# jovoy/SolarAxionRayTracing

Hardware: AMD Instinct MI355X
Metric: rays/sec (higher is better)
Workload: dtype f64

## Files before the change

### solaraxionraytracing_amd/csrc/sart_angular_scan.inc

```
  struct LdsLayout {
    TablesLds S;
    double cells[kRingExtraCells];
    DevBlob B;
    TraceArgs Ab;
    QueueLds<BLOCK / 64> Q;
  };
  __shared__ LdsLayout lds;
  static_assert((offsetof(LdsLayout, Q) % 512) == 0, "the rings are addressed with ds_*2st64 offsets");
  static_assert(kAScanCells == (BLOCK / 64) * kQueue, "the per-angle cells are the u5 column of the workgroup's rings");
  TablesLds& S = lds.S;
  QueueLds<BLOCK / 64>& Q = lds.Q;
  uint32_t* const cnt = reinterpret_cast<uint32_t*>(&lds.cells[kAScanCounters]);
  [[maybe_unused]] uint32_t* const cnt_out = reinterpret_cast<uint32_t*>(&lds.cells[kAImgNOutside]);
  auto acc_cell = [&](uint32_t t) -> double* { return &Q.w[t >> 7].u5[t & 127u]; };
  DevBlob& B = lds.B;
  TraceArgs& Ab = lds.Ab;
  (void)img_partials; (void)HBarg;
  {
    const uint64_t* src = reinterpret_cast<const uint64_t*>(blob);
    uint64_t* dst = reinterpret_cast<uint64_t*>(&B);
    for (int i = threadIdx.x; i < (int)(sizeof(DevBlob) / 8); i += BLOCK) dst[i] = src[i];
    if (threadIdx.x == 0) Ab = A;
    uint64_t* q = reinterpret_cast<uint64_t*>(&Q);
    for (int i = threadIdx.x; i < (int)(sizeof(Q) / 8); i += BLOCK) q[i] = 0ull;
// ... 128 lines not shown
    asm volatile("" :: "s"(HB.cdf_hi32), "s"(HB.energy_guide), "s"(HB.energy_tab), "s"(HB.refl), "s"(HB.refl_n_angles), "s"(HB.cdf_stride));
    RayOut out;
    phase_b<false, FAST, GAS, false, false, true>(Bo.P, L, HB, lds_opaque(Ab), st, e_idx, valid, out, nullptr);
    SART_STAGE_MARK("ACC");
    __builtin_amdgcn_s_setprio(SART_PRIO_ACC);
    if (__builtin_amdgcn_inverse_ballot_w64(out.m_nickel)) atomicAdd(&cnt[4 * kl + 1], 1u);
    if (__builtin_amdgcn_inverse_ballot_w64(out.m_till)) atomicAdd(&cnt[4 * kl + 2], 1u);
    if (out.passed) {
      atomicAdd(&cnt[4 * kl], 1u);
      double* const cell = acc_cell(kl * (2u * kScanLanes) + ((uint32_t)lane & (kScanLanes - 1u)));
      if constexpr (FIXED) {
        double fx_w, fx_w2;
        { const TraceArgs& Al = lds_opaque(Ab); fx_w = Al.fx_scale_w; fx_w2 = Al.fx_scale_w2; }
        __hip_atomic_fetch_add(reinterpret_cast<unsigned long long*>(cell), (unsigned long long)to_fixed(out.weight, fx_w), __ATOMIC_RELAXED,
                               __HIP_MEMORY_SCOPE_WORKGROUP);
        __hip_atomic_fetch_add(reinterpret_cast<unsigned long long*>(cell + kScanLanes), (unsigned long long)to_fixed(out.weight * out.weight, fx_w2),
                               __ATOMIC_RELAXED, __HIP_MEMORY_SCOPE_WORKGROUP);
      } else {
        __hip_atomic_fetch_add(cell, out.weight, __ATOMIC_RELAXED, __HIP_MEMORY_SCOPE_WORKGROUP);
        __hip_atomic_fetch_add(cell + kScanLanes, out.weight * out.weight, __ATOMIC_RELAXED, __HIP_MEMORY_SCOPE_WORKGROUP);
      }
      if constexpr (IMAGES) {
        SART_STAGE_MARK("IMG");
        TraceArgs Al;
        reload_kernarg(Al, offsetof(AScanKernArgs, A));
        asm volatile("" :: "s"(Al.replicas), "s"(Al.replica_stride), "s"(Al.image_nx), "s"(Al.image_ny), "s"(Al.image_x_min),
                     "s"(Al.image_y_min), "s"(Al.image_inv_step_x), "s"(Al.image_inv_step_y), "s"(Al.spectra));
        double* const blk = Al.replicas + (size_t)kl * (size_t)Al.replica_stride;
        double* const pos = &lds.cells[kAImgPos + kl * (3u * kAImgLanes) + ((uint32_t)lane & (kAImgLanes - 1u))];
        long long w_fx = 0;
        if constexpr (FIXED) {
          w_fx = to_fixed(out.weight, Al.fx_scale_w);
          __hip_atomic_fetch_add(reinterpret_cast<unsigned long long*>(pos), (unsigned long long)to_fixed(out.px, kFixedPositionScale),
                                 __ATOMIC_RELAXED, __HIP_MEMORY_SCOPE_WORKGROUP);
          __hip_atomic_fetch_add(reinterpret_cast<unsigned long long*>(pos + kAImgLanes), (unsigned long long)to_fixed(out.py, kFixedPositionScale),
                                 __ATOMIC_RELAXED, __HIP_MEMORY_SCOPE_WORKGROUP);
          __hip_atomic_fetch_add(reinterpret_cast<unsigned long long*>(pos + 2 * kAImgLanes), (unsigned long long)to_fixed(out.rdet, kFixedPositionScale),
                                 __ATOMIC_RELAXED, __HIP_MEMORY_SCOPE_WORKGROUP);
        } else {
          __hip_atomic_fetch_add(pos, out.px, __ATOMIC_RELAXED, __HIP_MEMORY_SCOPE_WORKGROUP);
          __hip_atomic_fetch_add(pos + kAImgLanes, out.py, __ATOMIC_RELAXED, __HIP_MEMORY_SCOPE_WORKGROUP);
          __hip_atomic_fetch_add(pos + 2 * kAImgLanes, out.rdet, __ATOMIC_RELAXED, __HIP_MEMORY_SCOPE_WORKGROUP);
        }
        const double fx = (out.px - Al.image_x_min) * Al.image_inv_step_x;
        const double fy = (out.py - Al.image_y_min) * Al.image_inv_step_y;
        const int nx = Al.image_nx, ny = Al.image_ny;
        const uint64_t inside_m = ballot64(fx >= 0.0) & ballot64(fx < (double)nx) & ballot64(fy >= 0.0) & ballot64(fy < (double)ny);
        if (__builtin_amdgcn_inverse_ballot_w64(inside_m)) {
          const uint32_t pix = (uint32_t)(int)fy * (uint32_t)nx + (uint32_t)(int)fx;
          if constexpr (FIXED) atomic_add_slot_i64(blk + pix, w_fx);
          else unsafeAtomicAdd(blk + pix, out.weight);
        } else {
          asm volatile("; rare: passed rays outside the image");
          atomicAdd(&cnt_out[kl], 1u);
          if constexpr (FIXED)
            __hip_atomic_fetch_add(reinterpret_cast<unsigned long long*>(&lds.cells[kAImgOutside + kl]), (unsigned long long)w_fx,
                                   __ATOMIC_RELAXED, __HIP_MEMORY_SCOPE_WORKGROUP);
        }
        if (Al.spectra) {
          double* rad = blk + (size_t)nx * (size_t)ny + SART_ACC_COUNT;
          double* en = rad + 2 * (size_t)Al.n_radial_bins;
          const size_t ne1 = (size_t)Pb.n_energies + 1;
          const int rb = min((int)(out.rdet * Al.radial_inv_bin), Al.n_radial_bins - 1);
          if constexpr (FIXED) {
            atomic_add_slot_i64(&rad[rb], 1);
            atomic_add_slot_i64(&rad[(size_t)Al.n_radial_bins + rb], w_fx);
            atomic_add_slot_i64(&en[out.e_idx], 1);
            atomic_add_slot_i64(&en[ne1 + out.e_idx], w_fx);
            atomic_add_slot_i64(&en[2 * ne1 + out.e_idx], to_fixed(out.reflect, kFixedReflectScale));
          } else {
            unsafeAtomicAdd(&rad[rb], 1.0);
            unsafeAtomicAdd(&rad[(size_t)Al.n_radial_bins + rb], out.weight);
            unsafeAtomicAdd(&en[out.e_idx], 1.0);
            unsafeAtomicAdd(&en[ne1 + out.e_idx], out.weight);
            unsafeAtomicAdd(&en[2 * ne1 + out.e_idx], out.reflect);
          }
        }
      }
    }
    __builtin_amdgcn_s_setprio(0);
  };

  constexpr bool kZonesInVgprs = FAST;
  uint32_t zone_lo_v[kMaxZones], zone_hi_v[kMaxZones];
#pragma unroll
  for (int z = 0; z < kMaxZones; ++z) {
    zone_lo_v[z] = H.zone_lo[z];
    zone_hi_v[z] = H.zone_hi[z];
    if (kZonesInVgprs) asm volatile("" : "+v"(zone_lo_v[z]), "+v"(zone_hi_v[z]));
  }
  uint32_t zone_reached_v = H.zone_reached;
  if (kZonesInVgprs) asm volatile("" : "+v"(zone_reached_v));
  uint32_t chunk = (uint32_t)wave_global;
  const uint32_t lane4 = 4u * (uint32_t)lane;
  uint32_t pass = 0;
  U4 stream = U4{0u, 0u, 0u, 0u};
  for (;;) {
    const bool have_new = chunk < n_chunks;
    SART_STAGE_MARK("LOOP");
    if (ka == n_angles) {
      if (have_new) {
        SART_STAGE_MARK("A0");
        if (pass == 0u) stream = stream_block(((first_chunk + (uint64_t)chunk) << 6) + (uint64_t)lane, A.seed_lo, A.seed_hi);
        const uint32_t w = word_of(stream, pass);
        const uint32_t rel = ((chunk << 8) + pass) + lane4;
        pass = (pass + 1u) & 3u;
        if (pass == 0u) chunk += (uint32_t)waves_total;
        if (early_reject) {
          ZoneTable Z;
          if constexpr (!kZonesInVgprs) reload_zones(Z);
          const uint32_t zone_reached = kZonesInVgprs ? (uint32_t)__builtin_amdgcn_readfirstlane((int)zone_reached_v) : Z.zone_reached;
          uint64_t dead_m = 0, reached_m = 0;
#pragma unroll
          for (int z = 0; z < kMaxZones; ++z) {
            const uint64_t in = kZonesInVgprs ? (ballot64(w >= zone_lo_v[z]) & ballot64(w <= zone_hi_v[z]))
                                              : (ballot64(w >= Z.lo[z]) & ballot64(w <= Z.hi[z]));
            dead_m |= in;
            reached_m |= ((zone_reached >> z) & 1u) ? in : 0ull;
          }
          const uint64_t valid_m = ballot64(rel >= rel_begin) & ballot64(rel < rel_end);
          n_reached += (uint32_t)__popcll(valid_m & reached_m);
          const uint64_t mask = valid_m & ~dead_m;
          if (__builtin_amdgcn_inverse_ballot_w64(mask)) {
            asm volatile("; hot: ring 0 write");
            const uint32_t slot = (t0 + prefix_of(mask)) % kQueue;
            Q.w[wave].ray[slot] = rel;
            Q.w[wave].u3hi[slot] = w;
          }
          t0 += (uint32_t)__popcll(mask);
          ring_sync();
        } else {
          run_bore(rel, (rel >= rel_begin) & (rel < rel_end), w);
        }
      }
      SART_STAGE_MARK("LOOP");
      if (early_reject) {
        const uint32_t n0 = t0 - h0;
        if ((n0 >= 64u) | (!have_new & (n0 > 0u))) {
          const uint32_t m = min(n0, 64u);
          const uint32_t slot = (h0 + (uint32_t)lane) % kQueue;
          const uint32_t rel = Q.w[wave].ray[slot];
          const uint32_t w = Q.w[wave].u3hi[slot];
          h0 += m;
          run_bore(rel, (uint32_t)lane < m, w);
        }
      }
    }
    SART_STAGE_MARK("LOOP");
    if (ka < n_angles) {
      run_telescope(ka);
      ++ka;
      ring_sync();
    }
    SART_STAGE_MARK("LOOP");
    const uint32_t n1 = t1 - h1;
    const bool draining = !have_new & (t0 == h0) & (ka == n_angles);
    if ((n1 >= 64u) | (draining & (n1 > 0u))) {
      run_mirrors(min(n1, 64u));
      ring_sync();
    }
    if (draining & (t1 == h1)) break;
  }

  SART_STAGE_MARK("EPILOGUE");
  if (lane == 0) atomicAdd(&cnt[4 * kAScanMaxAngles], n_reached);
  __syncthreads();
  using Sum = std::conditional_t<FIXED, long long, double>;
  for (int k = wave; k < n_angles; k += BLOCK / 64) {
    Sum* const dst = reinterpret_cast<Sum*>(ANarg.partials) + ((size_t)blockIdx.x * kAScanMaxAngles + (size_t)k) * kAScanPartialSlots;
    const double cell = *acc_cell((uint32_t)(k * 64 + lane));
    Sum v;
    if constexpr (FIXED) v = __double_as_longlong(cell); else v = cell;
#pragma unroll
    for (int off = 16; off > 0; off >>= 1) v += __shfl_xor(v, off, 64);
    if (lane == 0) dst[0] = v;
    if (lane == 32) dst[1] = v;
    if (lane < 4) dst[2 + lane] = (Sum)cnt[4 * k + lane];
    if (lane == 4) dst[6] = (k == 0) ? (Sum)cnt[4 * kAScanMaxAngles] : (Sum)0;
    if (lane == 5) dst[7] = (Sum)0;
    if constexpr (IMAGES) {
      const double pc = (lane < 3 * kAImgLanes) ? lds.cells[kAImgPos + k * (3 * kAImgLanes) + lane] : 0.0;
      Sum p;
      if constexpr (FIXED) p = __double_as_longlong(pc); else p = pc;
#pragma unroll
      for (int off = kAImgLanes / 2; off > 0; off >>= 1) p += __shfl_xor(p, off, 64);
      const Sum sw = __shfl(v, 0, 64), sw2 = __shfl(v, 32, 64);
      const Sum sx = __shfl(p, 0, 64), sy = __shfl(p, kAImgLanes, 64), sr = __shfl(p, 2 * kAImgLanes, 64);
      Sum s = 0;
      switch (lane) {
        case SART_ACC_SUM_WEIGHTS: s = sw; break;
        case SART_ACC_SUM_WEIGHTS_SQ: s = sw2; break;
        case SART_ACC_SUM_X: s = sx; break;
        case SART_ACC_SUM_Y: s = sy; break;
        case SART_ACC_SUM_R: s = sr; break;
        case SART_ACC_N_PASSED: s = (Sum)cnt[4 * k]; break;
        case SART_ACC_N_HIT_NICKEL: s = (Sum)cnt[4 * k + 1]; break;
        case SART_ACC_N_PASSED_TILL_WINDOW: s = (Sum)cnt[4 * k + 2]; break;
        case SART_ACC_N_SHELL_SELECTED: s = (Sum)cnt[4 * k + 3]; break;
        case SART_ACC_N_REACHED_TELESCOPE: s = (Sum)cnt[4 * kAScanMaxAngles]; break;
        case SART_ACC_N_OUTSIDE_IMAGE: s = (Sum)cnt_out[k]; break;
        case SART_ACC_SUM_WEIGHTS_OUTSIDE: if constexpr (FIXED) s = __double_as_longlong(lds.cells[kAImgOutside + k]); break;
        default: break;
// ... 5 lines not shown
```

### solaraxionraytracing_amd/csrc/sart_api.hip

```cpp
#include <hip/hip_runtime.h>
#include <rccl/rccl.h>
#include <dlfcn.h>
#include <sys/mman.h>
#include <unistd.h>

#include <algorithm>
#include <atomic>
#include <cmath>
#include <condition_variable>
#include <thread>
#include <cstdio>
#include <cstdlib>
#include <cstring>
#include <limits>
#include <map>
#include <mutex>
#include <string>
#include <vector>

#include "../../include/sart.h"
#include "sart_device.h"

namespace sart {
void launch_trace_histogram(const HotA& H, const HotB& HB, const DevBlob* blob, const TraceArgs& A, double* acc, int n_blocks,
                            hipStream_t stream, int variant, bool fixed);
void launch_finalize_fixed(const void* in, const void* hi, double* out, size_t n_img, int spectra, int n_radial_bins, int n_energies1, double q_w,
                           double q_w2, double q_pos, double q_refl, void* check_dev, hipStream_t stream);
void launch_rollover_fixed(void* acc, void* hi, size_t n, void* check_dev, hipStream_t stream);
size_t fixed_check_bytes();
std::string fixed_check_describe(const void* host_copy);
bool launch_trace_mass_scan(const HotA& H, const HotB& HB, const DevBlob* blob, const TraceArgs& A, const ScanArgs& SC, double* rows,
                            double* shared_row, int n_blocks, hipStream_t stream, int variant, bool fixed);
void launch_finalize_scan(const void* in, double* out, int n_masses, const double* q_w, const double* q_w2, int shared_row,
                          void* check_dev, hipStream_t stream, uint32_t counter_slots);
bool launch_trace_mass_scan_spectra(const HotA& H, const HotB& HB, const DevBlob* blob, const TraceArgs& A, const ScanArgs& SC, double* rows,
                                    double* shared_row, double* block0, double* counts, int n_blocks, hipStream_t stream, int variant, bool fixed);
int mass_scan_spectra_blocks_per_cu(int variant);
void launch_finalize_scan_bands(const void* rows, const void* shared_row, const void* in, double* out, const void* counts_in, double* counts_out,
                                int n_masses, int n_cells, const double* q_w, const double* q_w2, void* check_dev, hipStream_t stream);
void launch_trace_angular_scan(const HotA& H, const HotB& HB, const DevBlob* blob, const TraceArgs& A, const AScanArgs& AN, double* img_partials,
                               double* rows, double* shared_row, int n_blocks, hipStream_t stream, bool images, bool fast, bool fixed);
int angular_scan_blocks_per_cu(bool images, bool fast);
int energy_scan_blocks_per_cu(bool rotated);
void launch_trace_energy_scan(const HotA& H, const HotB& HB, const DevBlob* blob, const TraceArgs& A, const EScanArgs& EN, double* rows,
                              double* shared_row, int n_blocks, hipStream_t stream, bool rotated, bool fixed);
int shell_histogram_blocks_per_cu(bool rotated);
void launch_shell_histogram(const HotA& H, const HotB& HB, const DevBlob* blob, const TraceArgs& A, double* acc, const ShellArgs& SH,
                            int n_blocks, hipStream_t stream, bool rotated, bool fixed);
void launch_finalize_shells(const void* in, double* out, int n_shells, int n_energies1, int spectra, double q_w, double q_w2,
                            void* check_dev, hipStream_t stream);
int channel_histogram_blocks_per_cu(bool rotated);
void launch_channel_histogram(const HotA& H, const HotB& HB, const DevBlob* blob, const TraceArgs& A, double* acc, const ChannelArgs& CH,
                              int n_blocks, hipStream_t stream, bool rotated, bool fixed);
void launch_finalize_channels(const void* in, double* out, int n_channels, int n_energies1, int spectra, size_t n_img, double q_w,
                              double q_w2, void* check_dev, hipStream_t stream);
void launch_channel_fractions(const double* rates_dev, const double* total_dev, double* frac_dev, int n_channels, int stride,
                              size_t n_cells, unsigned long long* first_bad_dev, hipStream_t stream);
int origin_histogram_blocks_per_cu(bool rotated);
void launch_origin_histogram(const HotA& H, const HotB& HB, const DevBlob* blob, const TraceArgs& A, double* acc, const OriginArgs& OG,
                             int n_blocks, hipStream_t stream, bool rotated, bool fixed);
void launch_finalize_origin(const void* in, double* out, size_t n_cells, double q_w, double q_w2, void* check_dev, hipStream_t stream);
int aperture_histogram_blocks_per_cu(bool rotated);
void launch_aperture_histogram(const HotA& H, const HotB& HB, const DevBlob* blob, const TraceArgs& A, double* acc, const ApertureArgs& AP,
                               int n_blocks, hipStream_t stream, bool rotated, bool fixed);
int histogram_block_of(int variant);
void launch_trace_records(const HotA& H, const HotB& HB, const DevBlob* blob, const TraceArgs& A, sart_axion_t* out, int n_blocks,
                          hipStream_t stream, const double* uniforms_dev);
void launch_mirror_miss_count(const HotA& H, const DevBlob* blob, const TraceArgs& A, unsigned long long* counts, int n_blocks, hipStream_t stream);
void launch_radial_verdicts(const HotA& H, const DevBlob* blob, const double* radii, int n, uint32_t* out_table, uint32_t* out_compares,
                            hipStream_t stream);
int records_block();
int compact_chunk_max();
void launch_compact_records(const sart_axion_t* rec, uint32_t n, sart_axion_t* out, unsigned long long capacity, uint32_t* block_counts,
                            unsigned long long* block_first, unsigned long long* counts, hipStream_t stream);
void launch_stage_columns(const HotA& H, const HotB& HB, const DevBlob* blob, const TraceArgs& A, uint64_t* stage, uint32_t* flags,
                          uint32_t mask, int n_blocks, hipStream_t stream);
void launch_compact_columns(const uint64_t* stage, const uint32_t* flags, uint32_t n, uint32_t mask, unsigned long long ray_id0, uint64_t* out,
                            unsigned long long capacity, uint32_t* block_counts, unsigned long long* block_first,
                            unsigned long long* counts, hipStream_t stream);
int histogram_blocks_per_cu(int variant);
void launch_build_solar_tables(const double* em_dev, const double* radii_dev, const double* energies_dev, int n_radii, int n_energies,
                               double* cdf_dev, double* row_sum_dev, double* rcdf_dev, uint16_t* rguide_dev, uint16_t* eguide_dev,
                               uint32_t* status_dev, hipStream_t stream);
void launch_cdf_hi32(const double* cdf_dev, uint32_t* out_dev, size_t n, hipStream_t stream);
}

using namespace sart;

namespace {

thread_local std::string g_err;
int fail(int code, const std::string& msg) {
  g_err = msg;
  return code;
}
#define SART_HIP(call)                                                                              \
  do {                                                                                              \
    hipError_t e_ = (call);                                                                         \
    if (e_ != hipSuccess)                                                                           \
      return fail(e_ == hipErrorOutOfMemory ? SART_ERR_OUT_OF_MEMORY : SART_ERR_NO_DEVICE,          \
                  std::string(#call) + ": " + hipGetErrorString(e_));                               \
  } while (0)

constexpr double kPi = 3.14159265358979323846;
inline double deg2rad(double d) { return d * (kPi / 180.0); }
inline double cot(double x) { return 1.0 / std::tan(x); }

template <typename T>
struct DevBuf {
  T* p = nullptr;
  size_t n = 0;
  ~DevBuf() { if (p) (void)hipFree(p); }
  int upload(const T* host, size_t count) {
    if (count != n || !p) {
      if (p) (void)hipFree(p);
      p = nullptr; n = 0;
      SART_HIP(hipMalloc(reinterpret_cast<void**>(&p), count * sizeof(T)));
      n = count;
    }
    SART_HIP(hipMemcpy(p, host, count * sizeof(T), hipMemcpyHostToDevice));
    return 0;
  }
  int resize(size_t count) {
    if (count == n && p) return 0;
    if (p) (void)hipFree(p);
    p = nullptr; n = 0;
    SART_HIP(hipMalloc(reinterpret_cast<void**>(&p), count * sizeof(T)));
    n = count;
    return 0;
  }
  int reserve(size_t count) { return (p && n >= count) ? 0 : resize(count); }
  void release() {
    if (p) (void)hipFree(p);
    p = nullptr; n = 0;
  }
};

double linear1d(const std::vector<double>& xs, const std::vector<double>& ys, double x) {
  size_t lo = 0, hi = xs.size() - 1;
  while (hi - lo > 1) {
    const size_t mid = (lo + hi) / 2;
    if (xs[mid] <= x) lo = mid; else hi = mid;
  }
  return ys[lo] + (x - xs[lo]) * (ys[lo + 1] - ys[lo]) / (xs[lo + 1] - xs[lo]);
}

std::vector<double> sincos_table() {
  std::vector<double> t(2 * static_cast<size_t>(kSinCosEntries));
  const long double pi = 3.14159265358979323846264338327950288L;
  for (int k = 0; k < kSinCosEntries; ++k) {
    const int q = k / 32, j = k % 32;
    long double c, sn;
    if (j <= 16) { c = cosl(pi * j / 64); sn = sinl(pi * j / 64); }
// ... 479 lines not shown
HotA hot_of(const DevParams& P) {
  HotA h;
  std::memset(&h, 0, sizeof h);
  h.sun_distance = P.sun_distance; h.sun_radius = P.sun_radius;
  h.radius_cb = P.radius_cb; h.radius_cb_sq = P.radius_cb_sq; h.length_b = P.length_b; h.length_coldbore = P.length_coldbore;
  h.dz1 = P.length_coldbore - P.length_b;
  h.dz2 = h.dz1 + P.pipe1_len;
  h.dz3 = h.dz2 + P.pipe2_len;
  h.pipe1_radius_sq = P.pipe1_radius_sq;
  h.entrance_x = P.entrance_x; h.entrance_y = P.entrance_y;
  h.r1_last = P.r1_last; h.lut_inv_step = P.lut_inv_step;
  h.spider_z = P.spider_z; h.inner_radius = P.inner_radius;
  h.spoke_cos_thr = (P.spoke_n == 16) ? P.spoke_cos_thr * (1.0 / 32768.0) : P.spoke_cos_thr;
  h.ring_lo = P.ring_lo; h.ring_hi = P.ring_hi;
  h.test_active = P.test_active; h.rotated = P.rotated; h.telescope_kind = P.telescope_kind; h.spoke_n = P.spoke_n;
  h.n_shells = P.n_shells; h.lut_n = P.lut_n; h.radial_table = 0; h.inner_blocks = P.inner_blocks;
  return h;
}

double shell0_miss_radius_of(const sart_setup_t& s, const DevParams& P, int n_radii) {
  if (P.test_active || n_radii < 1) return -1.0;
  const double R = P.radius_cb;
  const double r_sun_max = (0.0015 + (n_radii - 1) * 0.0005) * P.sun_radius;
  const double s_max = (r_sun_max + R) / (P.sun_distance + P.length_b - r_sun_max) * (1.0 + 1e-6);
  if (P.telescope_wolter && s.n_shells > 0) {
    const double tilt = P.rotated ? std::acos(std::min(1.0, P.rx_c * P.ry_c)) : 0.0;
    const double s_tel = std::tan(std::atan(s_max) + tilt) * (1.0 + 1e-6);
    const double beta = s.all_angles_deg[0] * (kPi / 180.0), l = s.l_mirror, r1 = s.all_r1[0];
    const double tl = std::tan(beta) * l;
    const double r3 = -tl + std::sqrt(tl * tl + r1 * r1);
    return std::max(-1.0, r3 - s_tel * l * std::cos(beta) - 1e-3);
  }
  return -1.0;
}

struct MirrorMissBounds {
  float radius, slope_sq;
};
MirrorMissBounds mirror_miss_bounds_of(const sart_setup_t& s, const DevParams& P, const std::vector<ShellDev>& shells, int n_radii) {
  const MirrorMissBounds never = {std::numeric_limits<float>::infinity(), 0.0f};
  if (P.test_active || n_radii < 1 || !P.telescope_wolter || P.rotated || s.n_shells < 2) return never;
  const double R = P.radius_cb;
  const double r_sun_max = (0.0015 + (n_radii - 1) * 0.0005) * P.sun_radius;
  const double s_max = (r_sun_max + R) / (P.sun_distance + P.length_b - r_sun_max) * (1.0 + 1e-6);
  const HotA h = hot_of(P);
  const double l = P.l_mirror, zcb = -(h.dz3 - h.dz1), lz = l - zcb;
  if (!(l > 0.0) || !(zcb <= 0.0)) return never;
  const double eta = std::ldexp(1.0, -46), ulp16 = std::ldexp(1.0, -49);
  int j_min = s.n_shells;
  double m = s_max;
  for (int j = s.n_shells - 1; j >= 1; --j) {
    const ShellDev& sh = shells[static_cast<size_t>(j)];
    const double hb_max = sh.r1 * s_max + sh.m1_hb, hb_min = sh.m1_hb - sh.r1 * s_max, S = hb_max + s_max * sh.r1;
    const double moved = 4.0 * eta * l * S + ulp16 * (sh.r1 * sh.r1 + 2.0 * l * hb_max + s_max * l * s_max * l) +
                         std::fabs(sh.m1_cc - 2.0 * l * sh.m1_hb - sh.n1_r3sq);
    const bool a_ok = sh.m1_k == 0.0 && sh.m1_zhi <= l && hb_min > 1e-3 && kMirrorMissEps > 1e4 * moved;
    const double kappa = sh.n1_r3t / std::sqrt(sh.n1_r3sq + sh.n1_e * lz), num = sh.nickel_num;
    const double t = std::sqrt(num * num * (1.0 + 1e-6) / (lz * lz + num * num));
    const double m_j = kappa - t * std::sqrt((1.0 + kappa * kappa) * (1.0 + s_max * s_max));
    const bool b_ok = num > 0.0 && shells[static_cast<size_t>(j) - 1].r1 + zcb * s_max > 0.0 && m_j >= 0.4 * s_max;
    if (!(a_ok && b_ok)) break;
    m = std::min(m, m_j);
    j_min = j;
  }
  if (j_min >= s.n_shells) return never;
  MirrorMissBounds b;
  b.radius = static_cast<float>(shells[static_cast<size_t>(j_min) - 1].r1);
  if (static_cast<double>(b.radius) < shells[static_cast<size_t>(j_min) - 1].r1) b.radius = std::nextafterf(b.radius, std::numeric_limits<float>::infinity());
  b.slope_sq = static_cast<float>(m * m);
  if (static_cast<double>(b.slope_sq) > m * m) b.slope_sq = std::nextafterf(b.slope_sq, 0.0f);
  return b;
}

double tilt_bound_of(const sart_setup_t& s, double angle_y_deg) {
  const double t = std::fabs(deg2rad(s.telescope_turned_x_deg)) + std::fabs(deg2rad(angle_y_deg));
  if (t == 0.0) return 0.0;
  static const bool no_tilt_zones = std::getenv("SART_NO_TILT_ZONES") != nullptr;
  return no_tilt_zones ? -1.0 : t * (1.0 + 1e-9);
}

void build_zones(const sart_setup_t& s, const DevParams& P, int n_radii, HotA& h, double tilt_max) {
  h.n_zones = 0;
  h.zone_reached = 0;
  for (int z = 0; z < kMaxZones; ++z) { h.zone_lo[z] = 1u; h.zone_hi[z] = 0u; }
  if (P.test_active || n_radii < 1) return;
  const double R = P.radius_cb;
  const double r_sun_max = (0.0015 + (n_radii - 1) * 0.0005) * P.sun_radius;
  const double s_max = (r_sun_max + R) / (P.sun_distance + P.length_b - r_sun_max) * (1.0 + 1e-6);
  const double eps = 1e-6;
  const double dz[3] = {h.dz1, h.dz2, h.dz3};
  const double Rk[3] = {R, std::sqrt(P.pipe1_radius_sq), std::sqrt(P.pipe1_radius_sq)};
  double K_dead = 1e300;
  for (int k = 0; k < 3; ++k) K_dead = std::min(K_dead, Rk[k] + dz[k] * s_max + eps);
  double K_in = R - P.length_b * s_max - eps;
  for (int k = 0; k < 3; ++k) K_in = std::min(K_in, Rk[k] - dz[k] * s_max - eps);
  double spread = dz[2] * s_max + eps;
  const double gamma = std::atan(s_max) + tilt_max;
  const bool tilt_ok = tilt_max >= 0.0 && gamma < 0.5;
  if (tilt_max > 0.0 && tilt_ok) {
    const double h_tel = P.half_length_telescope;
    const double delta = 2.0 * std::sin(0.5 * tilt_max) * std::sqrt(Rk[2] * Rk[2] + h_tel * h_tel);
    spread += delta * (1.0 + std::tan(gamma)) * (1.0 + 1e-6) + eps;
  }
  struct Z { double lo, hi; bool reached; };
  std::vector<Z> zones;
  if (K_dead < R) zones.push_back({K_dead, 1e300, false});
  const bool on_axis = (P.entrance_x == 0.0 && P.entrance_y == 0.0) && tilt_ok;
  if (on_axis && K_in > 0) {
    auto add_reached = [&](double lo, double hi) {
      hi = std::min(hi, K_in);
      if (hi > lo) zones.push_back({lo, hi, true});
    };
    if (s.telescope_kind == SART_TK_XMM && P.inner_blocks > 0) add_reached(0.0, P.inner_radius - spread);
    if (s.telescope_kind == SART_TK_ABRIXAS) add_reached(0.0, P.inner_radius - spread);
    if (s.telescope_kind == SART_TK_XMM) add_reached(P.ring_lo + spread, P.ring_hi - spread);
    add_reached(P.r1_last + spread, std::min(K_in, K_dead));
  }
  for (const Z& z : zones) {
    if (h.n_zones >= kMaxZones) break;
    const double ulo = std::min(1.0, (z.lo / R) * (z.lo / R)), uhi = std::min(1.0, (z.hi / R) * (z.hi / R));
    const double wlo = std::ceil(ulo * 4294967296.0) + 1.0, whi = std::floor(uhi * 4294967296.0) - 2.0;
    if (!(whi >= wlo)) continue;
    h.zone_lo[h.n_zones] = static_cast<uint32_t>(std::min(wlo, 4294967295.0));
    h.zone_hi[h.n_zones] = static_cast<uint32_t>(std::min(whi, 4294967295.0));
    if (z.reached) h.zone_reached |= (1u << h.n_zones);
    h.n_zones++;
  }
}

double a0_survival_of(const HotA& h) {
  double covered = 0.0;
  for (int z = 0; z < h.n_zones; ++z) covered += static_cast<double>(h.zone_hi[z]) - static_cast<double>(h.zone_lo[z]) + 1.0;
  return std::min(1.0, std::max(0.0, 1.0 - covered / 4294967296.0));
}

constexpr double kA0WideMaxShare = 0.125;
double a0_wide_fallback_share(double s) {
  constexpr int W = 64, Q = 2 * W;
  if (!(s > 0.0)) return 0.0;
  s = std::min(s, 1.0);
  double pmf[W + 1];
  for (int k = 0; k <= W; ++k)
    pmf[k] = std::exp(std::lgamma(W + 1.0) - std::lgamma(k + 1.0) - std::lgamma(W - k + 1.0) + (k ? k * std::log(s) : 0.0) +
                      (k < W ? (W - k) * std::log1p(-s) : 0.0));
  auto pop = [](int x) { return x >= W ? x - W : x; };
  std::vector<double> T((W + 1) * (W + 1), 0.0), F(W + 1, 0.0);
  for (int n = 0; n <= W; ++n)
    for (int a = 0; a <= W; ++a)
      for (int b = 0; b <= W; ++b) {
        const double p = pmf[a] * pmf[b];
        const int n1 = n + a;
        if (n1 + b <= Q) T[n * (W + 1) + pop(n1 + b)] += p;
        else { F[n] += p; T[n * (W + 1) + pop(pop(n1) + b)] += p; }
      }
  std::vector<double> pi(W + 1, 1.0 / (W + 1)), next(W + 1);
  for (int it = 0; it < 20000; ++it) {
    std::fill(next.begin(), next.end(), 0.0);
    for (int n = 0; n <= W; ++n)
      for (int m = 0; m <= W; ++m) next[m] += pi[n] * T[n * (W + 1) + m];
    double d = 0.0;
    for (int m = 0; m <= W; ++m) d += std::fabs(next[m] - pi[m]);
    pi.swap(next);
    if (d < 1e-13) break;
  }
  double share = 0.0;
  for (int n = 0; n <= W; ++n) share += pi[n] * F[n];
  return share;
}
bool a0_wide_rule(double survival) { return a0_wide_fallback_share(survival) <= kA0WideMaxShare; }

bool path_is_constant(const DevParams& P, const HotA& h, int n_radii) {
  if (P.test_active || n_radii < 1) return false;
  const double R = P.radius_cb;
  const double r_sun_max = (0.0015 + (n_radii - 1) * 0.0005) * P.sun_radius;
  const double s_max = (r_sun_max + R) / (P.sun_distance + P.length_b - r_sun_max) * (1.0 + 1e-6);
  const double dz[3] = {h.dz1, h.dz2, h.dz3};
  const double Rk[3] = {R, std::sqrt(P.pipe1_radius_sq), std::sqrt(P.pipe1_radius_sq)};
  double reach = 1e300;
  for (int k = 0; k < 3; ++k) reach = std::min(reach, Rk[k] + (P.length_b + dz[k]) * s_max);
  return reach + 1e-6 < R;
}

uint32_t radial_verdict_of(const HotA& H, const DevParams& P, const std::vector<ShellDev>& shells, const uint8_t* lut, bool cand_on, double radial,
                           bool* both = nullptr) {
  auto cell_of = [&](double r) {
    const double x = r * H.lut_inv_step;
    return !(x >= 0.0) ? 0 : (x >= static_cast<double>(H.lut_n - 1)) ? H.lut_n - 1 : static_cast<int>(x);
  };
  bool ok = true;
  if (H.telescope_kind != SART_TK_LLNL) {
    const bool inner = (H.telescope_kind == SART_TK_XMM) ? (radial <= H.inner_radius) : (radial < H.inner_radius);
    const bool ring = (H.telescope_kind == SART_TK_XMM) & (radial < H.ring_hi) & (radial > H.ring_lo);
    ok = !(inner | ring);
  }
  ok = ok & !(radial > H.r1_last);
  const int nS = H.n_shells;
  const int j0 = lut[cell_of(radial)];
  const int jc = std::min(j0, nS - 1), jb = std::max(jc - 1, 0);
  const double c_r1 = shells[jc].r1, c_ro = shells[jc].r1_outer;
  const double b_r1 = shells[jb].r1, b_ro = shells[jb].r1_outer;
  const bool step = (j0 < nS) & !(c_r1 > radial);
  const int j = j0 + (step ? 1 : 0);
  ok = ok & (j < nS);
  const double g_r1 = step ? c_r1 : b_r1, g_ro = step ? c_ro : b_ro;
  ok = ok & !((j > 0) & (radial > g_r1) & (radial < g_ro));
  const uint32_t shell = static_cast<uint32_t>(std::min(j, nS - 1));
  const bool below0 = radial < P.shell0_miss_radius, cand = cand_on & (radial > static_cast<double>(P.mirror_miss_radius));
  if (both) *both = ok & below0 & cand;
  const uint32_t code = !ok ? 0u : below0 ? 1u : cand ? 3u : 2u;
  return code << 6 | shell;
}

bool build_radial_table(sart_context* c) {
  std::fill(c->shell_lut.begin() + kRadialCellsOffset, c->shell_lut.end(), static_cast<uint8_t>(0));
  c->radial_n = 0;
// ... 608 lines not shown
  c->n_radii = nR;
  c->n_energies = nE;
  c->have_solar = true;
  c->derived_dirty = true;
  return 0;
}

static_assert(kEnergyGuideEntries == 2594 && kRadiusGuideEntries == 3074, "include/sart.h (sart_get_solar_tables) and _lib.py (ENERGY_GUIDE_ENTRIES, RADIUS_GUIDE_ENTRIES) state these numbers");
int sart_get_solar_tables(sart_context* c, double* rcdf_out, double* ecdf_out, uint16_t* radius_guide_out, uint16_t* energy_guide_out) {
  if (!c) return fail(SART_ERR_INVALID_ARGUMENT, "ctx is NULL");
  if (!c->have_solar) return fail(SART_ERR_NOT_READY, "no solar tables");
  SART_HIP(hipSetDevice(c->device));
  SART_HIP(hipStreamSynchronize(c->stream));
  const size_t nR = static_cast<size_t>(c->n_radii), nE = static_cast<size_t>(c->n_energies);
  if (rcdf_out) SART_HIP(hipMemcpy(rcdf_out, c->d_rcdf.p, nR * sizeof(double), hipMemcpyDeviceToHost));
  if (ecdf_out)
    SART_HIP(hipMemcpy2D(ecdf_out, nE * sizeof(double), c->d_ecdf.p, (nE + kEnergyCdfPad) * sizeof(double), nE * sizeof(double), nR,
                         hipMemcpyDeviceToHost));
  if (radius_guide_out) SART_HIP(hipMemcpy(radius_guide_out, c->d_rguide.p, kRadiusGuideEntries * sizeof(uint16_t), hipMemcpyDeviceToHost));
  if (energy_guide_out) SART_HIP(hipMemcpy(energy_guide_out, c->d_eguide.p, nR * kEnergyGuideEntries * sizeof(uint16_t), hipMemcpyDeviceToHost));
  return 0;
}

int sart_set_reflectivity(sart_context* c, int32_t nC, int32_t nA, int32_t nE, double amin, double amax, double emin,
                          double emax, const double* data) {
  if (!c || !data) return fail(SART_ERR_INVALID_ARGUMENT, "NULL argument");
  if (nC < 1 || nC > SART_MAX_COATINGS || nA < 2 || nE < 2 || !(amax > amin) || !(emax > emin))
    return fail(SART_ERR_INVALID_ARGUMENT, "invalid reflectivity grid");
  c->refl_data.assign(data, data + static_cast<size_t>(nC) * nA * nE);
  c->refl_nc = nC; c->refl_na = nA; c->refl_ne = nE;
  c->refl_amin = amin; c->refl_amax = amax; c->refl_emin = emin; c->refl_emax = emax;
  c->have_refl = true;
  c->derived_dirty = true;
  return 0;
}

int sart_set_detector_tables(sart_context* c, const double* sbx, const double* sby, int32_t nsb, const double* wx,
                             const double* wy, int32_t nw, const double* gx, const double* gy, int32_t ng) {
  if (!c || !sbx || !sby || !wx || !wy || !gx || !gy) return fail(SART_ERR_INVALID_ARGUMENT, "NULL argument");
  if (nsb < 2 || nw < 2 || ng < 2) return fail(SART_ERR_INVALID_ARGUMENT, "tables need at least two points");
  auto ascending = [](const double* x, int n) { for (int i = 1; i < n; ++i) if (!(x[i] > x[i - 1])) return false; return true; };
  if (!ascending(sbx, nsb) || !ascending(wx, nw) || !ascending(gx, ng))
    return fail(SART_ERR_INVALID_ARGUMENT, "table abscissae must be strictly ascending");
  c->sb_x.assign(sbx, sbx + nsb); c->sb_y.assign(sby, sby + nsb);
  c->win_x.assign(wx, wx + nw); c->win_y.assign(wy, wy + nw);
  c->gas_x.assign(gx, gx + ng); c->gas_y.assign(gy, gy + ng);
  c->have_det = true;
  c->derived_dirty = true;
  return 0;
}

static int trace_records_impl(sart_context* c, const sart_trace_params_t* p, sart_axion_t* out_dev, const double* uniforms_dev) {
  if (!c || !out_dev) return fail(SART_ERR_INVALID_ARGUMENT, "NULL argument");
  SART_HIP(hipSetDevice(c->device));
  if (int rc = launch_record_rays(c, p, [&](const TraceArgs& a, int n_blocks) {
        launch_trace_records(c->hot, c->hotb, c->d_blob.p, a, out_dev, n_blocks, c->stream, uniforms_dev);
      }))
    return rc;
  SART_HIP(hipGetLastError());
  return 0;
}

int sart_trace_records_device(sart_context* c, const sart_trace_params_t* p, sart_axion_t* out_dev) {
  return trace_records_impl(c, p, out_dev, nullptr);
}

__attribute__((visibility("default"))) int sart_internal_trace_records_uniforms(sart_context* c, const sart_trace_params_t* p,
                                                                               const double* uniforms_host, sart_axion_t* out_host) {
  if (!c || !p || !uniforms_host || !out_host) return fail(SART_ERR_INVALID_ARGUMENT, "NULL argument");
  if (p->n_rays == 0) return 0;
  SART_HIP(hipSetDevice(c->device));
  DevBuf<double> d_u;
  if (int rc = d_u.upload(uniforms_host, 6 * p->n_rays)) return rc;
  if (int rc = c->d_rec.reserve(p->n_rays)) return rc;
  if (int rc = trace_records_impl(c, p, c->d_rec.p, d_u.p)) return rc;
  SART_HIP(hipMemcpyAsync(out_host, c->d_rec.p, p->n_rays * sizeof(sart_axion_t), hipMemcpyDeviceToHost, c->stream));
  SART_HIP(hipStreamSynchronize(c->stream));
  return 0;
}

__attribute__((visibility("default"))) int sart_internal_zones(sart_context* c, uint32_t* lo, uint32_t* hi, uint32_t* reached_bits) {
  if (!c || !lo || !hi || !reached_bits) return -1;
  if (hipSetDevice(c->device) != hipSuccess || refresh_derived(c) != 0 || sync_blob(c) != 0) return -1;
  for (int z = 0; z < c->hot.n_zones; ++z) { lo[z] = c->hot.zone_lo[z]; hi[z] = c->hot.zone_hi[z]; }
  *reached_bits = c->hot.zone_reached & ((1u << kMaxZones) - 1u);
  return c->hot.n_zones;
}

__attribute__((visibility("default"))) double sart_internal_a0_wide_share(double survival) { return a0_wide_fallback_share(survival); }
__attribute__((visibility("default"))) int sart_internal_a0_wide_rule(double survival) { return a0_wide_rule(survival) ? 1 : 0; }
__attribute__((visibility("default"))) int sart_internal_a0_wide(sart_context* c, double* survival) {
  if (!c || !survival) return -1;
  if (hipSetDevice(c->device) != hipSuccess || refresh_derived(c) != 0 || sync_blob(c) != 0) return -1;
  *survival = c->hot.n_zones > 0 ? a0_survival_of(c->hot) : 1.0;
  return (c->hot.zone_reached >> kA0WideBit) & 1u;
}

__attribute__((visibility("default"))) int sart_internal_shell0_miss_radius(sart_context* c, double* out) {
  if (!c || !out) return fail(SART_ERR_INVALID_ARGUMENT, "NULL argument");
  SART_HIP(hipSetDevice(c->device));
  if (int rc = refresh_derived(c)) return rc;
  if (int rc = sync_blob(c)) return rc;
  *out = c->params.shell0_miss_radius;
  return 0;
}

__attribute__((visibility("default"))) int sart_internal_mirror_miss(sart_context* c, const sart_trace_params_t* params, double* radius,
                                                                     double* slope_sq, double* thresholds, unsigned long long* counts) {
  if (!c || !radius || !slope_sq) return fail(SART_ERR_INVALID_ARGUMENT, "NULL argument");
  SART_HIP(hipSetDevice(c->device));
  if (int rc = refresh_derived(c)) return rc;
  if (int rc = sync_blob(c)) return rc;
  const double rmin = c->params.mirror_miss_radius;
  *radius = rmin;
  *slope_sq = c->params.mirror_miss_slope_sq;
  if (thresholds) {
    for (int j = 0; j < c->setup.n_shells; ++j) {
      const ShellDev& sh = c->shells[static_cast<size_t>(j)];
      const bool on = j > 0 && sh.r1 > rmin;
      thresholds[j] = on ? sh.n1_r3sq - kMirrorMissEps : -std::numeric_limits<double>::infinity();
    }
  }
  if (counts) {
    TraceArgs a;
    if (int rc = make_args(c, params, a)) return rc;
    DevBuf<unsigned long long> d_counts;
    const unsigned long long zero[5] = {0, 0, 0, 0, 0};
    if (int rc = d_counts.upload(zero, 5)) return rc;
    if (a.n_rays > 0)
      launch_mirror_miss_count(c->hot, c->d_blob.p, a, d_counts.p, grid_for(a.n_rays, c->n_cu, 4, records_block()), c->stream);
    SART_HIP(hipGetLastError());
    SART_HIP(hipMemcpyAsync(counts, d_counts.p, sizeof zero, hipMemcpyDeviceToHost, c->stream));
    SART_HIP(hipStreamSynchronize(c->stream));
  }
  return 0;
}

int sart_get_radial_table(sart_context* c, double* breakpoints, uint32_t* verdicts, uint8_t* cells, int32_t* n_cells) {
  if (!c) return fail(SART_ERR_INVALID_ARGUMENT, "ctx is NULL");
  SART_HIP(hipSetDevice(c->device));
  if (int rc = refresh_derived(c)) return rc;
  if (int rc = sync_blob(c)) return rc;
  if (n_cells) *n_cells = c->params.lut_n;
  if (c->radial_n > 0) {
    const uint8_t* t = c->shell_lut.data() + kRadialTableOffset;
    if (breakpoints) std::memcpy(breakpoints, t + offsetof(RadialLds, b), static_cast<size_t>(c->radial_n) * sizeof(double));
    if (verdicts) std::memcpy(verdicts, t + offsetof(RadialLds, w), static_cast<size_t>(c->radial_n) * sizeof(uint32_t));
    if (cells) std::memcpy(cells, c->shell_lut.data() + kRadialCellsOffset, static_cast<size_t>(c->params.lut_n));
  }
  return c->radial_n;
}

__attribute__((visibility("default"))) int sart_internal_radial_verdicts(sart_context* c, const double* radii, int32_t n, uint32_t* by_table,
                                                                         uint32_t* by_compares) {
  if (!c || !radii || !by_table || !by_compares || n < 1) return fail(SART_ERR_INVALID_ARGUMENT, "invalid argument");
  SART_HIP(hipSetDevice(c->device));
  if (int rc = refresh_derived(c)) return rc;
  if (int rc = sync_blob(c)) return rc;
  if (!c->hot.radial_table) return fail(SART_ERR_UNSUPPORTED, "this setup has no radial verdict table");
  DevBuf<double> d_r;
  DevBuf<uint32_t> d_out;
  if (int rc = d_r.upload(radii, static_cast<size_t>(n))) return rc;
  if (int rc = d_out.resize(2 * static_cast<size_t>(n))) return rc;
  launch_radial_verdicts(c->hot, c->d_blob.p, d_r.p, n, d_out.p, d_out.p + n, c->stream);
  SART_HIP(hipGetLastError());
  SART_HIP(hipMemcpyAsync(by_table, d_out.p, static_cast<size_t>(n) * sizeof(uint32_t), hipMemcpyDeviceToHost, c->stream));
  SART_HIP(hipMemcpyAsync(by_compares, d_out.p + n, static_cast<size_t>(n) * sizeof(uint32_t), hipMemcpyDeviceToHost, c->stream));
  SART_HIP(hipStreamSynchronize(c->stream));
  return 0;
// ... 278 lines not shown
  c->d_rec.release();
  c->d_rec2.release();
  c->d_cmp.release();
  c->d_col_stage.release();
  c->d_col_flags.release();
  for (auto& b : c->d_col_cmp) b.release();
  return 0;
}

namespace {

size_t shell_block_len_of(const sart_context* c, const sart_trace_params_t* p) {
  return sart_shell_block_len(c->setup.n_shells, c->n_energies, p->spectra);
}

size_t channel_block_len_of(const sart_context* c, const sart_trace_params_t* p) {
  return sart_channel_block_len(c->n_channels, c->n_energies, p->spectra, p->image_nx, p->image_ny);
}

size_t origin_block_len_of(const sart_context* c, const sart_trace_params_t*) { return sart_origin_block_len(c->n_radii, c->n_energies); }

size_t aperture_block_len_of(const sart_context* c, const sart_trace_params_t*) {
  return sart_aperture_block_len(c->aperture_grid.nx, c->aperture_grid.ny);
}

struct Breakdown {
  int tile_max, tile_extra_max;
  size_t partial_slots;
  DevBuf<double> sart_context::*partials;
  int (sart_context::*blocks_per_cu)[2];
  int (*kernel_blocks_per_cu)(bool rotated);
  size_t (*block_len)(const sart_context* c, const sart_trace_params_t* p);
  void (*launch)(sart_context* c, const TraceArgs& a, double* acc_dev, double* block_dev, int n_blocks, bool rotated, bool fixed);
  int (*check)(sart_context* c, const sart_trace_params_t* p);
  DevBuf<double> sart_context::*block;
  DevBuf<double> sart_context::*block_fin;
  int (*finalize)(sart_context* c, const sart_trace_params_t* p, const void* raw_dev, double* out_dev);
};
struct BreakdownBlock {
  const Breakdown* kind = nullptr;
  double* dev = nullptr;
};

int histogram_launch(sart_context* c, const sart_trace_params_t* p, double* acc_dev, BreakdownBlock bd = {}) {
  SART_HIP(hipSetDevice(c->device));
  if (int rc = refresh_derived(c)) return rc;
  if (int rc = sync_blob(c)) return rc;
  TraceArgs a;
  if (int rc = make_args(c, p, a)) return rc;
  const bool fixed = c->accum_mode == SART_ACCUM_FIXED64 && !c->tile.in_pilot;
  a.fx_scale_w = a.fx_scale_w2 = 0.0;
  if (fixed) {
    if (int rc = freeze_quanta(c, weight_bound_of(c, p->flags, c->params.gas_dm2_abs), !p->accumulate)) return rc;
    a.fx_scale_w = std::ldexp(1.0, -c->weight_exp);
    a.fx_scale_w2 = std::ldexp(1.0, -c->weight_sq_exp);
  }
  if (!p->accumulate) SART_HIP(hipMemsetAsync(acc_dev, 0, acc_len_of(c, p) * sizeof(double), c->stream));
  if (bd.kind && !p->accumulate) SART_HIP(hipMemsetAsync(bd.dev, 0, bd.kind->block_len(c, p) * sizeof(double), c->stream));
  if (a.n_rays == 0) return 0;
  if (a.n_rays > (1ull << 31)) {
    sart_trace_params_t q = *p;
    q.accumulate = 1;
    for (uint64_t done = 0; done < p->n_rays;) {
      const uint64_t n = std::min<uint64_t>(p->n_rays - done, 1ull << 31);
      q.n_rays = n;
      q.ray_id_offset = p->ray_id_offset + done;
      if (int rc = histogram_launch(c, &q, acc_dev, bd)) return rc;
      done += n;
    }
    return 0;
  }
  const int variant = hist_variant_of(c);
  {
    const sart_setup_t& s = c->setup;
    const double spot_px = s.distance_detector_xrt * (0.25 * s.radius_sun / s.distance_sun_earth) *
                           a.image_inv_step_x;
    int R = spot_px > 96.0 ? 8 : 64;
    if (static_cast<size_t>(p->image_nx) * static_cast<size_t>(p->image_ny) > (1u << 20)) R = std::min(R, 1);
    if (s.test_active) R = 64;
    if (c->knobs.image_replicas > 0) R = std::min(kMaxImageReplicas, c->knobs.image_replicas);
    if (c->tile.in_pilot) R = 64;
    if (p->image_nx == 0) R = 1;
    while (R & (R - 1)) R &= R - 1;
    if (R > 1) {
      const size_t n_img = static_cast<size_t>(p->image_nx) * static_cast<size_t>(p->image_ny);
      const size_t pad = 32;
      if (n_img + pad > 0xFFFFFFFFull) return fail(SART_ERR_INVALID_ARGUMENT, "image too large for replicated accumulation");
      a.replica_stride = static_cast<uint32_t>(n_img + pad);
      const size_t need = static_cast<size_t>(R) * (n_img + pad);
      DevBuf<double>& reps = c->tile.in_pilot ? c->d_pilot_replicas : c->d_replicas;
      if (reps.n != need || !reps.p) {
        SART_HIP(hipStreamSynchronize(c->stream));
        if (int rc = reps.resize(need)) return rc;
        SART_HIP(hipMemsetAsync(reps.p, 0, need * sizeof(double), c->stream));
      }
      a.replicas = reps.p;
      a.replica_mask = static_cast<uint32_t>(R - 1);
      const bool ring_cells_free = c->hot.n_zones == 0 || variant == 5 || variant == 6;
      if (!c->knobs.no_image_tile && !c->tile.in_pilot) {
        sart_context::TileCache& t = c->tile;
        const bool same = t.valid && t.nx == p->image_nx && t.ny == p->image_ny && t.x_min == p->image_x_min &&
                          t.x_max == p->image_x_max && t.y_min == p->image_y_min && t.y_max == p->image_y_max &&
                          t.ring_cells_free == ring_cells_free;
        if (!same) {
          t.valid = false;
          t.n = 0;
          sart_trace_params_t q = *p;
          q.n_rays = 200000;
          q.image_nx = q.image_ny = 1;
          q.accumulate = 0;
          q.spectra = 0;
          if (int rc = c->d_pilot.resize(sart_accumulator_len(1, 1))) return rc;
          t.in_pilot = true;
          const bool was_timing = c->timing;
          c->timing = false;
          const int rc = sart_trace_histogram_device(c, &q, c->d_pilot.p);
          c->timing = was_timing;
          t.in_pilot = false;
          if (rc) return rc;
          double sc[SART_ACC_COUNT];
          SART_HIP(hipMemcpyAsync(sc, c->d_pilot.p + 1, sizeof sc, hipMemcpyDeviceToHost, c->stream));
          SART_HIP(hipStreamSynchronize(c->stream));
          t.nx = p->image_nx; t.ny = p->image_ny;
          t.x_min = p->image_x_min; t.x_max = p->image_x_max; t.y_min = p->image_y_min; t.y_max = p->image_y_max;
          t.ring_cells_free = ring_cells_free;
          if (sc[SART_ACC_N_PASSED] >= 100.0) {
            const double cx = (sc[SART_ACC_SUM_X] / sc[SART_ACC_N_PASSED] - p->image_x_min) * a.image_inv_step_x;
            const double cy = (sc[SART_ACC_SUM_Y] / sc[SART_ACC_N_PASSED] - p->image_y_min) * a.image_inv_step_y;
            int n = std::min({static_cast<int>(ring_cells_free ? kImageTileMax : kImageTileExtraMax), p->image_nx, p->image_ny});
            if (c->knobs.image_tile_max > 0) n = std::min(n, c->knobs.image_tile_max);
            const int x0 = std::clamp(static_cast<int>(std::floor(cx)) - n / 2, 0, p->image_nx - n);
            const int y0 = std::clamp(static_cast<int>(std::floor(cy)) - n / 2, 0, p->image_ny - n);
            t.x0 = x0; t.y0 = y0; t.n = n;
          }
          t.valid = true;
        }
        a.tile_x0 = t.x0; a.tile_y0 = t.y0; a.tile_n = t.n;
        a.tile_base = ring_cells_free ? 0 : kTileRingCells;
        if (bd.kind) {
          const bool free_s = c->hot.n_zones == 0;
          const int n = std::min(t.n, free_s ? bd.kind->tile_max : bd.kind->tile_extra_max);
          a.tile_x0 = t.x0 + (t.n - n) / 2; a.tile_y0 = t.y0 + (t.n - n) / 2; a.tile_n = n;
          a.tile_base = free_s ? 0 : kTileRingCells;
        }
      }
    } else {
      a.replicas = acc_dev;
      a.replica_mask = 0u;
    }
  }
  if (bd.kind) {
    const bool rotated = c->params.rotated != 0;
    int& bpc = (c->*bd.kind->blocks_per_cu)[rotated];
    if (bpc == 0) {
      bpc = std::max(1, bd.kind->kernel_blocks_per_cu(rotated));
      if (c->knobs.hist_blocks_per_cu > 0) bpc = c->knobs.hist_blocks_per_cu;
    }
    const int n_blocks = grid_for(a.n_rays, c->n_cu, bpc, 1024);
    const size_t rows = std::max<size_t>(static_cast<size_t>(n_blocks), static_cast<size_t>(c->n_cu) * 4);
    if (c->d_partials.n < static_cast<size_t>(n_blocks) * SART_ACC_COUNT) {
      SART_HIP(hipStreamSynchronize(c->stream));
      if (int rc = c->d_partials.resize(rows * SART_ACC_COUNT)) return rc;
    }
    DevBuf<double>& table_partials = c->*bd.kind->partials;
    if (table_partials.n < static_cast<size_t>(n_blocks) * bd.kind->partial_slots) {
      SART_HIP(hipStreamSynchronize(c->stream));
// ... 1324 lines not shown
```

### solaraxionraytracing_amd/csrc/sart_device.h

```cpp
#pragma once
#include <stdint.h>

namespace sart {

constexpr int kMaxShells = 64;
constexpr int kMaxStrips = 16;
constexpr int kRadiusGuide = 2048;
constexpr int kRadiusGuideTop = 1024;
constexpr uint32_t kRadiusGuideTopStart = 0xF8000000u;
constexpr int kRadiusGuideEntries = kRadiusGuide + 1 + kRadiusGuideTop + 1;
#ifndef SART_ENERGY_GUIDE_DIV
#define SART_ENERGY_GUIDE_DIV 1024
#endif
constexpr int kEnergyGuideDiv = SART_ENERGY_GUIDE_DIV;
constexpr int kEnergyGuideUniform = kEnergyGuideDiv / 32 * 31;
constexpr int kEnergyGuideLogMax = 25 * 64;
constexpr int kEnergyGuideBuckets = kEnergyGuideUniform + kEnergyGuideLogMax + 1;
constexpr int kEnergyGuideEntries = kEnergyGuideBuckets + 1;
constexpr uint32_t kEnergyGuideCode0 = (1023u - 5u) << 6;
constexpr int kEnergyCdfPad = 4;
constexpr int kShellLutMax = 1024;
constexpr int kMaxRadii = 2048;
constexpr int kSinCosEntries = 129;

// ... 2 lines not shown
  double r1_outer;
  double m1_k, m1_hb, m1_cc, m1_zhi;
  double m2_k, m2_hb, m2_cc, m2_zlo, m2_zhi;
  double m2_rc;
  double n1_tan;
  double n1_r3t;
  double n1_r3sq, n1_e;
  double n2_tan;
  double n2_r3t;
  double n2_r3sq, n2_e, n2_invF;
  double dist_det, dist_det_end;
  double dist_det_raw;
  double nickel_num;
  int32_t coating;
  int32_t refl_row0;
};
static_assert(sizeof(ShellDev) % 8 == 0, "ShellDev is staged into LDS as 8-byte words");

struct EnergyDev {
  double energy;
  double t_window;
  double t_strongback;
  double a_gas;
  double gamma;
  double inv_two_e_ev;
  double mu_pipe;
  double mu_magnet;
};

struct DevParams {
  double sun_distance, sun_radius;
  double radius_cb, radius_cb_sq, length_b, length_coldbore;
  double pipe1_len, pipe2_len, pipe1_radius_sq;
  int32_t n_radii, n_energies;
  int32_t radius_span;
  int32_t lut_n;
  int32_t test_active, test_parallel;
  double test_x, test_y, test_z, test_radius, test_radius_sq, test_collimator_z;
  int32_t telescope_wolter;
  int32_t telescope_kind;
  int32_t n_shells, rotated;
  double l_mirror;
  double rx_c, rx_s, ry_c, ry_s, half_length_telescope;
  double entrance_x, entrance_y;
  double r1_last;
  double lut_inv_step;
  float mirror_miss_radius, mirror_miss_slope_sq;
  double shell0_miss_radius;
  double spider_z;
  double inner_radius;
  double ring_lo, ring_hi;
  int32_t spoke_n;
  int32_t inner_blocks;
  double spoke_cos_thr;
  int32_t hole_type, number_of_holes;
  double hole_in_optics;
  double pipe_c, pipe_s, d_cb_xray;
  double lateral_shift, transversal_shift;
  double radius_window_sq, chip_cx, chip_cy;
  double theta_c, theta_s;
  int32_t n_half_strips, stage_gas;
  double strip_lo[kMaxStrips], strip_hi[kMaxStrips];
  double conv_k;
  double exposure;
  double gas_m_gamma_sq, gas_term1, gas_inv_hbarc_m;
  double gas_dm2_abs;
  int32_t refl_n_angles, n_coatings;
  double refl_angle_min, refl_inv_dangle, refl_dangle;
};
static_assert(sizeof(DevParams) < 2048, "DevParams travels in the kernel-argument segment");

struct HotA {
  double sun_distance, sun_radius;
  double radius_cb, radius_cb_sq, length_b, length_coldbore;
  double dz1, dz2, dz3;
  double pipe1_radius_sq;
  double entrance_x, entrance_y;
  double r1_last, lut_inv_step;
  double spider_z, spoke_cos_thr, inner_radius, ring_lo, ring_hi;
  int32_t test_active, rotated, telescope_kind, spoke_n;
  int32_t n_shells, lut_n, radial_table, inner_blocks;
  int32_t n_zones;
  uint32_t zone_reached;
  uint32_t zone_lo[4], zone_hi[4];
};
constexpr int kMaxZones = 4;
constexpr int kA0WideBit = 8;
constexpr uint32_t kA0WideMask = 0x5u << kA0WideBit;
static_assert(kA0WideBit >= kMaxZones, "the wide-pass switch lies above the zones' bits");

struct HotB {
  const double* diff_flux_cdfs;
  const uint32_t* cdf_hi32;
  const uint16_t* energy_guide;
  const EnergyDev* energy_tab;
  const double* refl;
  int32_t n_energies, refl_n_angles;
  int32_t cdf_stride, _pad;
};

struct DevTables {
  const double* sincos_tab;
  const ShellDev* shells;
  const uint8_t* shell_lut;
  const double* flux_radius_cdf;
  const uint16_t* radius_guide;
  const double* diff_flux_cdfs;
  const uint16_t* energy_guide;
  const EnergyDev* energy_tab;
  const double* refl;
};

struct DevBlob {
  DevParams P;
  DevTables T;
};
static_assert(sizeof(DevBlob) % 8 == 0, "DevBlob is staged into LDS as 8-byte words");

constexpr int kMaxImageReplicas = 128;

struct TraceArgs {
  uint64_t n_rays, ray_id_offset;
  double* replicas;
  uint32_t replica_mask;
  uint32_t replica_stride;
  double* partials;
  uint32_t seed_lo, seed_hi;
  uint32_t flags;
  int32_t image_nx, image_ny;
  double image_x_min, image_y_min, image_inv_step_x, image_inv_step_y;
  int32_t spectra, n_radial_bins;
  double radial_inv_bin;
  int32_t tile_x0, tile_y0, tile_n, tile_base;
  double fx_scale_w, fx_scale_w2;
};
constexpr int kScanMaxMasses = 32;
constexpr int kScanLanes = 32;
struct ScanMass {
  double dm2_abs;
  double fx_scale_w, fx_scale_w2;
  uint32_t aux[2];
};
struct ScanArgs {
  int32_t n_masses;
  int32_t n_bands;
  double* partials;
  ScanMass m[kScanMaxMasses];
};
static_assert(sizeof(ScanMass) == 32 && offsetof(ScanMass, aux) == 24 && sizeof(ScanArgs) == 16 + 32 * kScanMaxMasses,
              "the kernel re-reads ScanArgs with scalar loads at these offsets");
constexpr int kScanPartialSlots = 4;
constexpr int kScanBandSlots = (kScanMaxMasses + 1) * 2 * kScanLanes;
constexpr int kScanBandsMax = kScanLanes - 1;

constexpr int kAScanMaxAngles = 32;
struct AScanAngle {
  double rx_c, rx_s, ry_c, ry_s, half_length_telescope;
  double shell0_miss_radius;
  double mx, my, mz;
  double _pad;
};
struct AScanArgs {
  int32_t n_angles, _pad;
  double* partials;
  AScanAngle a[kAScanMaxAngles];
};
static_assert(sizeof(AScanAngle) == 80 && sizeof(AScanArgs) == 16 + 80 * kAScanMaxAngles, "the kernel re-reads AScanArgs with scalar loads at these offsets");
// ... 103 lines not shown
```

### solaraxionraytracing_amd/csrc/sart_kernels.hip

```cpp
#include <hip/hip_runtime.h>
#include <stdint.h>
#include <string.h>

#include <type_traits>

#include "../../include/sart.h"
#include "sart_device.h"
#include "sart_math.h"

namespace sart {

struct U4 { uint32_t x, y, z, w; };
constexpr int kPhiloxRounds = 7;

__device__ __forceinline__ U4 philox4x32(uint32_t c0, uint32_t c1, uint32_t c2, uint32_t c3, uint32_t k0,
                                         uint32_t k1) {
#pragma unroll
  for (int r = 0; r < kPhiloxRounds; ++r) {
    const uint64_t p0 = (uint64_t)0xD2511F53u * c0;
    const uint64_t p1 = (uint64_t)0xCD9E8D57u * c2;
    const uint32_t hi0 = (uint32_t)(p0 >> 32), lo0 = (uint32_t)p0;
    const uint32_t hi1 = (uint32_t)(p1 >> 32), lo1 = (uint32_t)p1;
    const uint32_t n0 = __builtin_amdgcn_bitop3_b32(hi1, c1, k0, 0x96);
    const uint32_t n2 = __builtin_amdgcn_bitop3_b32(hi0, c3, k1, 0x96);
    c0 = n0; c1 = lo1; c2 = n2; c3 = lo0;
    k0 += 0x9E3779B9u;
    k1 += 0xBB67AE85u;
  }
  return U4{c0, c1, c2, c3};
}

__device__ __forceinline__ U4 stream_block(uint64_t group, uint32_t k0, uint32_t k1) {
  return philox4x32((uint32_t)group, (uint32_t)(group >> 32), 3u, 0u, k0, k1);
}
__device__ __forceinline__ uint32_t word_of(const U4& b, uint32_t k) {
  return k == 0u ? b.x : (k == 1u ? b.y : (k == 2u ? b.z : b.w));
}

#define SART_STAGE_MARK(name) asm volatile("; SART_STAGE " name)

__device__ __forceinline__ uint64_t ballot64(bool pred) { return __builtin_amdgcn_ballot_w64(pred); }

template <uint64_t BITS>
__device__ __forceinline__ double scalar_const() {
  uint32_t lo, hi;
  asm volatile("s_mov_b32 %0, %2\n\ts_mov_b32 %1, %3" : "=s"(lo), "=s"(hi) : "n"((uint32_t)BITS), "n"((uint32_t)(BITS >> 32)));
  return __longlong_as_double((long long)(((uint64_t)hi << 32) | (uint64_t)lo));
}
#define SC(x) (scalar_const<__builtin_bit_cast(uint64_t, (double)(x))>())

__device__ __forceinline__ double fma_vvs(double p, double x, double c_scalar) {
  double r;
  asm("v_fma_f64 %0, %1, %2, %3" : "=v"(r) : "v"(p), "v"(x), "s"(c_scalar));
  return r;
}
#define HORNER(p, x, c) fma_vvs((p), (x), (double)(c))

__device__ __forceinline__ double u52(uint32_t hi, uint32_t lo) {
  const uint32_t mlo = __builtin_amdgcn_alignbit(hi, lo, 12u);
  const uint32_t mhi = __builtin_amdgcn_alignbit(0x3FFu, hi, 12u);
  return __longlong_as_double((long long)(((uint64_t)mhi << 32) | (uint64_t)mlo)) - 1.0;
}

struct SinCosCoef { double s3, s2, s1, s0, d3, d2, d1; };
__device__ __forceinline__ SinCosCoef sincos_coef() {
  return SinCosCoef{SC(-0.5992645293207921), SC(2.5501640398773455), SC(-5.16771278004997), SC(3.141592653589793),
                    SC(-1.3352627688545895), SC(4.0587121264167685), SC(-4.934802200544679)};
}
template <int TURNS>
__device__ __forceinline__ void sincos_turns(double u, const double* __restrict__ table, const SinCosCoef& K, double* sn, double* cs) {
  constexpr double T = (double)TURNS;
  const double kf = __builtin_rint(u * (64.0 * T));
  const double r = fma(-1.0 / 64.0, kf, u * T);
  const double2 t = reinterpret_cast<const double2*>(table)[(int)kf];
  const double x = r * r;
  const double sr = fma(fma(fma(K.s3, x, K.s2), x, K.s1), x, K.s0) * r;
  const double cr = fma(fma(fma(K.d3, x, K.d2), x, K.d1), x, 1.0);
  *sn = fma(t.x, sr, t.y * cr);
  *cs = fma(-t.y, sr, t.x * cr);
}

__device__ __forceinline__ double asin_small(double x, double x2) {
  double p = 0.01396484375;
  p = HORNER(p, x2, 0.017352764423076924);
  p = HORNER(p, x2, 0.022372159090909092);
  p = HORNER(p, x2, 0.030381944444444444);
  p = HORNER(p, x2, 0.044642857142857144);
  p = HORNER(p, x2, 0.075);
  p = HORNER(p, x2, 0.16666666666666666);
  double r = fma(x * x2, p, x);
  if (!(fabs(x) < 0.06)) {
    asm volatile("; rare: asin outside the series' range");
    r = asin(x);
  }
  return r;
}

__device__ __forceinline__ void asin_small_pair(double xa, double xa2, double xb, double xb2, double& ra, double& rb) {
  double pa = 0.01396484375, pb = 0.01396484375;
#define SART_STEP2(c) pa = HORNER(pa, xa2, c); pb = HORNER(pb, xb2, c)
  SART_STEP2(0.017352764423076924);
  SART_STEP2(0.022372159090909092);
  SART_STEP2(0.030381944444444444);
  SART_STEP2(0.044642857142857144);
  SART_STEP2(0.075);
  SART_STEP2(0.16666666666666666);
#undef SART_STEP2
  ra = fma(xa * xa2, pa, xa);
  rb = fma(xb * xb2, pb, xb);
  if (!(fabs(xa) < 0.06)) {
    asm volatile("; rare: asin outside the series' range");
    ra = asin(xa);
  }
  if (!(fabs(xb) < 0.06)) {
    asm volatile("; rare: asin outside the series' range");
    rb = asin(xb);
  }
}

__device__ __forceinline__ double atan_small(double x) {
  const double x2 = x * x;
  double p = -1.0 / 15.0;
  p = fma(p, x2, 1.0 / 13.0);
  p = fma(p, x2, -1.0 / 11.0);
// ... 607 lines not shown
    const bool xmm = H.telescope_kind == SART_TK_XMM;
    uint64_t blocked_m = (xmm ? ballot64(inner_le) : ballot64(inner_lt)) | (xmm ? (ballot64(ring_a) & ballot64(ring_b)) : 0ull) |
                         ballot64(spoke_a) | ballot64(spoke_b);
    if (cfg_holes) {
      const int nH = P.number_of_holes;
      const int lim = nH - (int)ceil((double)nH / 2.0);
      bool res = false, done = false;
      for (int l = -lim; l <= lim; ++l) {
        double hx = 0.0, hy = 0.0;
        if (l != 0) {
          if ((abs(l) & 1) == 0) hy += 2.0 * (double)l * P.hole_in_optics;
          else hx += 2.0 * ((double)l + ((double)l / (double)abs(l))) * P.hole_in_optics;
        }
        const double ix = X0 - hx, iy = Y0 - hy, rad = P.hole_in_optics;
        const double tx = ix / sqrt(2.0) - iy / sqrt(2.0), ty = ix / sqrt(2.0) + iy / sqrt(2.0);
        const double axx = fabs(ix), ayy = fabs(iy), atx = fabs(tx), aty = fabs(ty);
        bool through = false;
        switch (P.hole_type) {
          case SART_HT_CIRCLE: through = sqrt(fma(ix, ix, iy * iy)) < rad; break;
          case SART_HT_CROSS:
            through = (axx < rad && ayy < rad * 16.0) || (ayy < rad && axx < rad * 16.0); break;
          case SART_HT_STAR:
            through = (axx < rad && ayy < rad * 16.0) || (ayy < rad && axx < rad * 16.0) ||
                      (atx < rad && aty < rad * 16.0) || (aty < rad && atx < rad * 16.0); break;
          case SART_HT_SQUARE: through = axx < rad && ayy < rad; break;
          case SART_HT_DIAMOND: through = atx < rad && aty < rad; break;
          default: through = false;
        }
        if (!done) { res = !through; done = through; }
      }
      if (inner) blocked = res;
      blocked_m = ballot64(blocked);
    }
    ok = ok & !blocked;
    okm &= ~blocked_m;
  }

  const bool beyond = radial > H.r1_last;
  ok = ok & !beyond;
  okm &= ~ballot64(beyond);
  const int nS = H.n_shells;
  const int j0 = (int)L.lut[max(min((int)(radial * H.lut_inv_step), H.lut_n - 1), 0)];
  const int jc = min(j0, nS - 1), jb = max(jc - 1, 0);
  const double c_r1 = L.shells[jc].r1, c_ro = L.shells[jc].r1_outer;
  const double b_r1 = L.shells[jb].r1, b_ro = L.shells[jb].r1_outer;
  const bool step = (j0 < nS) & !(c_r1 > radial);
  const int j = j0 + (step ? 1 : 0);
  const bool has_shell = j < nS;
  ok = ok & has_shell;
  okm &= ballot64(has_shell);
  const double g_r1 = step ? c_r1 : b_r1, g_ro = step ? c_ro : b_ro;
  const bool gf_a = j > 0, gf_b = radial > g_r1, gf_c = radial < g_ro;
  ok = ok & !(gf_a & gf_b & gf_c);
  const uint64_t step_m = ballot64(j0 < nS) & ~ballot64(c_r1 > radial);
  const uint64_t in_c = ballot64(radial > c_r1) & ballot64(radial < c_ro), in_b = ballot64(radial > b_r1) & ballot64(radial < b_ro);
  okm &= ~(ballot64(gf_a) & ((step_m & in_c) | (~step_m & in_b)));
  M.ok = okm;
  st.shell = min(j, nS - 1);
  radial_out = radial;
  if (r3sq) {
    const double c_r3sq = L.shells[jc].n1_r3sq, u_r3sq = L.shells[jc + 1].n1_r3sq;
    *r3sq = step ? u_r3sq : c_r3sq;
  }
  if constexpr (RTAB) {
    M.keep = ~ballot64(radial < P.shell0_miss_radius);
    M.cand = (ROT != 0) ? 0ull : ballot64(radial > (double)P.mirror_miss_radius);
  }
  return ok;
}

template <bool FAST, int ROT, bool ZEXT, bool NOWALL = false, bool WORD = false, bool RTAB = false>
__device__ __forceinline__ bool phase_a_core(const HotA& H, const DevParams& P, const LdsTables& L, const Uniforms& U, RayState& st,
                                             bool& sampled, bool& reached, double& radial_out, LaneMasks& M, const SinCosCoef* held = nullptr,
                                             double* r3sq = nullptr) {
  static_assert(!ZEXT || (FAST && ROT == 0), "the z-extent form needs the magnet-frame slopes in phase B");
  static_assert(!NOWALL || ZEXT, "the constant-path form is a specialisation of the vacuum, unrotated one");
  BoreRay br;
  phase_a_bore<FAST, ZEXT, NOWALL, WORD>(H, P, L, U, st, sampled, reached, br, M, held);
  return phase_a_telescope<FAST, ROT, RTAB>(H, P, tel_rot_of(P), L, br, st, radial_out, M, r3sq);
}

__device__ __forceinline__ Uniforms uniforms_of(uint32_t seed_lo, uint32_t seed_hi, uint64_t ray_id, uint32_t u3_hi) {
  const uint32_t id_lo = (uint32_t)ray_id, id_hi = (uint32_t)(ray_id >> 32);
  const U4 b0 = philox4x32(id_lo, id_hi, 0u, 0u, seed_lo, seed_hi);
  Uniforms U;
  U.u2 = u52(b0.x, 0u);
  U.u2_hi = b0.x;
  U.u5 = u52(b0.z, 0u);
  U.u5_hi = b0.z;
  U.u0 = u52(b0.y & 0xFFFFF800u, 0u);
  U.u1 = u52(b0.w & 0xFFFFF800u, 0u);
  U.u4 = u52((b0.y << 21) | ((b0.w & 0x7FFu) << 10), 0u);
  U.u3 = u52(u3_hi, 0u);
  return U;
}
template <bool FAST, int ROT, bool ZEXT, bool NOWALL = false, bool WORD = true, bool RTAB = false>
__device__ __forceinline__ bool phase_a(const HotA& H, const DevParams& P, const LdsTables& L, uint32_t seed_lo,
                                        uint32_t seed_hi, uint64_t ray_id, uint32_t u3_hi, RayState& st, bool& sampled,
                                        bool& reached, double& radial, LaneMasks& M, const SinCosCoef* held = nullptr,
                                        double* r3sq = nullptr) {
  return phase_a_core<FAST, ROT, ZEXT, NOWALL, WORD, RTAB>(H, P, L, uniforms_of(seed_lo, seed_hi, ray_id, u3_hi), st, sampled, reached, radial, M, held, r3sq);
}

__device__ __forceinline__ double zcb_rotated(double mx, double my, double mz, double h, double qx, double qy, double tsx, double tsy, double Lp) {
  const double num = -Lp - h - fma(mx, qx, fma(my, qy, -mz * h));
  return num * frcp(fma(mx, tsx, fma(my, tsy, mz)));
}

struct RayOut {
  uint64_t m_nickel = 0, m_till = 0, m_passed = 0;
  bool passed = false;
#ifdef SART_STAGE_TIMING
  uint64_t tb[6] = {0, 0, 0, 0, 0, 0};
#endif
  double px = 0.0, py = 0.0, rdet = 0.0, weight = 0.0, reflect = 0.0;
  int e_idx = 0;
  GasRay gas = {0.0, 0.0, 0.0, 0.0, 0.0};
};

#ifndef SART_GATHER_LIVE
#define SART_GATHER_LIVE 1
#endif
#ifndef SART_B_LIVE_REGION
#define SART_B_LIVE_REGION 1
#endif
#ifndef SART_A_SINCOS_VGPR
#define SART_A_SINCOS_VGPR 1
#endif
struct EScanGeo {
  double cos_ya, path_cb, distance_pipe_m, xu1, xu2;
  int ia1, ia2;
  uint64_t m_live;
  uint64_t m_chip;
  uint64_t m_strip;
};
template <bool RECORDS, bool FAST, int GAS, bool ZEXT, bool SCAN = false, bool NODRAW = false, bool ESCAN = false>
__device__ __forceinline__ void phase_b(const DevParams& P, const LdsTables& L, const HotB& HB, const TraceArgs& A,
                                        const RayState& st, int e_idx_in, bool live, RayOut& out, sart_axion_t* rec,
                                        EScanGeo* geo = nullptr) {
#ifdef SART_STAGE_TIMING
#define SART_B_STAMP(k, dep) do { asm volatile("" :: "v"(dep)); out.tb[k] = __builtin_readcyclecounter(); } while (0)
#else
#define SART_B_STAMP(k, dep)
#endif
  SART_B_STAMP(0, st.X0);
  constexpr bool WORD = !RECORDS;
  const bool draw_energy = NODRAW ? false : __builtin_amdgcn_readfirstlane(e_idx_in) < 0;
  EnergyDraw ed = {};
#ifdef SART_DEBUG_KNOBS
  const uint32_t dbg = (uint32_t)__builtin_amdgcn_readfirstlane((int)A.flags);
  if (draw_energy) energy_draw_begin<WORD>(HB, (dbg & 0x02000000u) ? (st.r_idx & 15) : st.r_idx, st.u5, st.u5_hi, ed, (dbg & 0x04000000u) ? (st.r_idx & 15) : st.r_idx);
#else
  if (draw_energy) energy_draw_begin<WORD>(HB, st.r_idx, st.u5, st.u5_hi, ed);
#endif
  const ShellDev& sh = L.shells[st.shell];
  const int wolter = __builtin_amdgcn_readfirstlane(P.telescope_wolter);
  static_assert(!ZEXT || GAS >= 0, "the z-extent form needs the stage at compile time");
  static_assert(!SCAN || !RECORDS, "the mass scan accumulates, it writes no records");
  const int stage_gas = (GAS >= 0) ? GAS : __builtin_amdgcn_readfirstlane(P.stage_gas);
  const int test_active = FAST ? 0 : __builtin_amdgcn_readfirstlane(P.test_active);
  const int n_half_strips = __builtin_amdgcn_readfirstlane(P.n_half_strips);
  const uint32_t flags = (uint32_t)__builtin_amdgcn_readfirstlane((int)A.flags);
  const double X0 = st.X0, Y0 = st.Y0, tsx = st.tsx, tsy = st.tsy, zcb = st.zcb;
  const double Q0 = fma(X0, X0, Y0 * Y0);

  const double D0 = fma(X0, tsx, Y0 * tsy);
  const double A0 = fma(tsx, tsx, tsy * tsy);
// ... 249 lines not shown
    out.rdet = fsqrt_pos(r_rdet2 + 1e-300);
    if constexpr (SCAN) out.gas = r_gas;
    out.passed = __builtin_amdgcn_inverse_ballot_w64(out.m_passed);
    out.px = -r_pdx + P.chip_cx;
    out.py = r_pdy + P.chip_cy;
  } else {
    behind_the_mirrors();
  }
}

#ifndef SART_PRIO_A1
#define SART_PRIO_A1 2
#endif
#ifndef SART_PRIO_B
#define SART_PRIO_B 3
#endif
#ifndef SART_PRIO_ACC
#define SART_PRIO_ACC 1
#endif
constexpr int kQueue = 128;

struct __align__(16) TablesLds {
  double sincos[2 * kSinCosEntries];
  uint32_t rcdf_hi[kMaxRadii + 4];
  ShellDev shells[kMaxShells];
  uint16_t rguide[kRadiusGuideEntries + 6];
  uint8_t lut[kShellLutMax];
};

struct __align__(16) WaveRings {
  double X0[kQueue], Y0[kQueue], tsx[kQueue], tsy[kQueue];
  double path[kQueue], u5[kQueue];
  int idx[kQueue];
  uint32_t ray[kQueue];
  uint32_t u3hi[kQueue];
};
struct __align__(16) HistRings {
  double X0[kQueue], Y0[kQueue], tsx[kQueue], tsy[kQueue];
  double path[kQueue];
  uint2 cell[kQueue];
  uint32_t ray[kQueue];
  uint32_t u3hi[kQueue];
};
static_assert(sizeof(WaveRings) - sizeof(HistRings) == kQueue * sizeof(uint32_t) && sizeof(HistRings) % 512 == 0 &&
                  (kTileRingCells / kQueue * (sizeof(WaveRings) - sizeof(HistRings))) / sizeof(double) == kTileExtraCells + kRadialTableCells - kRingExtraCells,
              "what ring 1's packed cell frees is what the histogram kernels' image tile grows by");
template <int WAVES, typename Rings = WaveRings>
struct __align__(16) QueueLds {
  Rings w[WAVES];
};

template <int BLOCK>
__device__ __forceinline__ void stage_tables(TablesLds& S, const DevParams& P, const DevTables& T, bool radial_cells = false) {
  for (int i = threadIdx.x; i < 2 * kSinCosEntries; i += BLOCK) S.sincos[i] = as_global(T.sincos_tab)[i];
  for (int i = threadIdx.x; i < P.n_radii + 4; i += BLOCK) {
    const double c = (i < P.n_radii) ? as_global(T.flux_radius_cdf)[i] : 1.0;
    const unsigned long long t = __double2ull_rd(c * 4503599627370496.0) >> 20;
    S.rcdf_hi[i] = t > 0xFFFFFFFFull ? 0xFFFFFFFFu : (uint32_t)t;
  }
  for (int i = threadIdx.x; i < kRadiusGuideEntries; i += BLOCK) S.rguide[i] = as_global(T.radius_guide)[i];
  {
    const auto src = as_global(reinterpret_cast<const uint64_t*>(T.shells));
    uint64_t* dst = reinterpret_cast<uint64_t*>(S.shells);
    const int n = P.n_shells * (int)(sizeof(ShellDev) / 8);
    for (int i = threadIdx.x; i < n; i += BLOCK) dst[i] = src[i];
  }
  const uint8_t* lut = T.shell_lut + (radial_cells ? kRadialCellsOffset : 0);
  for (int i = threadIdx.x; i < P.lut_n; i += BLOCK) S.lut[i] = as_global(lut)[i];
  __syncthreads();
}

__device__ __forceinline__ void reload_hot(HotA& dst) {
  typedef const __attribute__((address_space(4))) uint32_t* kernarg_ptr;
  kernarg_ptr p = (kernarg_ptr)__builtin_amdgcn_kernarg_segment_ptr();
  asm volatile("" : "+s"(p));
  uint32_t* d = reinterpret_cast<uint32_t*>(&dst);
#pragma unroll
  for (int k = 0; k < (int)(sizeof(HotA) / 4); ++k) d[k] = p[k];
}

struct ZoneTable {
  int32_t n_zones;
  uint32_t zone_reached;
  uint32_t lo[kMaxZones], hi[kMaxZones];
};
static_assert(sizeof(ZoneTable) == sizeof(HotA) - offsetof(HotA, n_zones), "ZoneTable mirrors the tail of HotA");
static_assert(offsetof(WaveRings, u3hi) == offsetof(WaveRings, ray) + kQueue * sizeof(uint32_t) && offsetof(WaveRings, ray) % 8 == 0 &&
                  offsetof(HistRings, u3hi) == offsetof(HistRings, ray) + kQueue * sizeof(uint32_t) && offsetof(HistRings, ray) % 8 == 0,
              "the image tile uses ray + u3hi of every wave as 128 contiguous doubles");
__device__ __forceinline__ void reload_zones(ZoneTable& dst) {
  typedef const __attribute__((address_space(4))) uint32_t* kernarg_ptr;
  kernarg_ptr p = (kernarg_ptr)__builtin_amdgcn_kernarg_segment_ptr() + offsetof(HotA, n_zones) / 4;
  asm volatile("" : "+s"(p));
  uint32_t* d = reinterpret_cast<uint32_t*>(&dst);
#pragma unroll
  for (int k = 0; k < (int)(sizeof(ZoneTable) / 4); ++k) d[k] = p[k];
}

struct HistKernArgs {
  HotA H;
  const DevBlob* blob;
  TraceArgs A;
  double* acc;
  HotB HB;
  ScanArgs SC;
};
static_assert(offsetof(HistKernArgs, H) == 0 && offsetof(HistKernArgs, blob) == (sizeof(HotA) + 7) / 8 * 8 &&
                  offsetof(HistKernArgs, A) == offsetof(HistKernArgs, blob) + 8 &&
                  offsetof(HistKernArgs, acc) == offsetof(HistKernArgs, A) + sizeof(TraceArgs) &&
                  offsetof(HistKernArgs, HB) == offsetof(HistKernArgs, acc) + 8 &&
                  offsetof(HistKernArgs, SC) == offsetof(HistKernArgs, HB) + sizeof(HotB) && sizeof(HotA) % 4 == 0 &&
                  sizeof(TraceArgs) % 8 == 0 && sizeof(HotB) % 8 == 0,
              "reload_hot / reload_zones / reload_kernarg read the arguments at these offsets");
template <typename T>
__device__ __forceinline__ void reload_kernarg(T& dst, size_t byte_offset) {
  static_assert(sizeof(T) % 4 == 0, "dword granularity");
  typedef const __attribute__((address_space(4))) uint32_t* kernarg_ptr;
  kernarg_ptr p = (kernarg_ptr)__builtin_amdgcn_kernarg_segment_ptr() + byte_offset / 4;
  asm volatile("" : "+s"(p));
  uint32_t* d = reinterpret_cast<uint32_t*>(&dst);
#pragma unroll
  for (int k = 0; k < (int)(sizeof(T) / 4); ++k) d[k] = p[k];
}

template <int BLOCK, bool FAST, bool ROT, int GAS, bool PATHC, bool FIXED, bool SCAN = false>
__global__ __launch_bounds__(BLOCK) void trace_histogram_kernel(HotA H, const DevBlob* __restrict__ blob, TraceArgs A,
                                                                double* __restrict__ acc, HotB HBarg, ScanArgs SCarg) {
  constexpr bool BANDS = false;
#include "sart_trace_histogram.inc"
}
template <int BLOCK, bool FAST, bool ROT, int GAS, bool PATHC, bool FIXED>
__global__ __launch_bounds__(BLOCK) void mass_scan_spectra_kernel(HotA H, const DevBlob* __restrict__ blob, TraceArgs A,
                                                                  double* __restrict__ acc, HotB HBarg, ScanArgs SCarg) {
  constexpr bool SCAN = true, BANDS = true;
#include "sart_trace_histogram.inc"
}

struct ShellKernArgs {
  HotA H;
  const DevBlob* blob;
  TraceArgs A;
  double* acc;
  HotB HB;
  ShellArgs SH;
};
static_assert(offsetof(ShellKernArgs, A) == offsetof(HistKernArgs, A) && offsetof(ShellKernArgs, HB) == offsetof(HistKernArgs, HB) &&
                  offsetof(ShellKernArgs, SH) == offsetof(HistKernArgs, SC),
              "the shell kernel shares the argument offsets of the histogram kernel");
static_assert(kShellImageTileMax * kShellImageTileMax <= kTileRingCells + kRingExtraCells - kShellTableCells &&
                  kShellImageTileExtraMax * kShellImageTileExtraMax <= kRingExtraCells - kShellTableCells,
              "the shell kernel's image tile leaves the shell table alone");

struct ChanKernArgs {
  HotA H;
  const DevBlob* blob;
  TraceArgs A;
  double* acc;
  HotB HB;
  ChannelArgs CH;
};
static_assert(offsetof(ChanKernArgs, A) == offsetof(HistKernArgs, A) && offsetof(ChanKernArgs, HB) == offsetof(HistKernArgs, HB) &&
                  offsetof(ChanKernArgs, CH) == offsetof(HistKernArgs, SC),
              "the channel kernel shares the argument offsets of the histogram kernel");

struct OriginKernArgs {
  HotA H;
  const DevBlob* blob;
  TraceArgs A;
// ... 357 lines not shown
          atomic_add_slot_i64(oc + SART_ORIGIN_N, 1);
          atomic_add_slot_i64(oc + SART_ORIGIN_SUM_WEIGHTS, w_fx);
          atomic_add_slot_i64(oc + SART_ORIGIN_SUM_WEIGHTS_SQ, w2_fx);
        } else {
          unsafeAtomicAdd(oc + SART_ORIGIN_N, 1.0);
          unsafeAtomicAdd(oc + SART_ORIGIN_SUM_WEIGHTS, out.weight);
          unsafeAtomicAdd(oc + SART_ORIGIN_SUM_WEIGHTS_SQ, out.weight * out.weight);
        }
      }
      if constexpr (kAperture) {
        reload_kernarg(BDl, BD::kArgsOffset);
        double* const ac = BDl.block + SART_APERTURE_HEAD + (size_t)ap_cell * SART_APERTURE_CELL;
        if constexpr (FIXED) {
          atomic_add_slot_i64(ac + SART_APERTURE_N, 1);
          atomic_add_slot_i64(ac + SART_APERTURE_SUM_WEIGHTS, w_fx);
          atomic_add_slot_i64(ac + SART_APERTURE_SUM_WEIGHTS_SQ, w2_fx);
        } else {
          unsafeAtomicAdd(ac + SART_APERTURE_N, 1.0);
          unsafeAtomicAdd(ac + SART_APERTURE_SUM_WEIGHTS, out.weight);
          unsafeAtomicAdd(ac + SART_APERTURE_SUM_WEIGHTS_SQ, out.weight * out.weight);
        }
      }
      if constexpr (kChannels) {
        const uint32_t cl = (uint32_t)lane & (uint32_t)(kChanLanes - 1);
        const size_t c_ne1 = (size_t)BDl.n_energies1, c_nimg = (size_t)nx * (size_t)ny;
        double* const c_en = BDl.block + (size_t)BDl.n_channels * SART_CHAN_ROW;
        double* const c_img = c_en + (Al.spectra ? (size_t)BDl.n_channels * c_ne1 : (size_t)0);
        if (BDl.stride == 8) {
#pragma unroll
          for (int k = kMaxChannels / 4; k < kMaxChannels / 2; ++k) {
            const d2 v = gload<d2>(BDl.frac, f_off + 16u * (uint32_t)k);
            f[2 * k] = v.x;
            f[2 * k + 1] = v.y;
          }
        }
#pragma unroll
        for (int t = 0; t < kMaxChannels; ++t) {
          if (t >= BDl.n_channels) break;
          const double ft = f[t];
          if (ft > 0.0) __hip_atomic_fetch_add(&lds.tab.cnt[t][cl], 1u, __ATOMIC_RELAXED, __HIP_MEMORY_SCOPE_WORKGROUP);
          const double c = out.weight * ft;
          if (c != 0.0) {
            if constexpr (FIXED) {
              const long long c_fx = to_fixed(c, Al.fx_scale_w);
              const long long c2_fx = to_fixed(c * c, Al.fx_scale_w2);
              __hip_atomic_fetch_add(reinterpret_cast<unsigned long long*>(&lds.tab.sum[t][0][cl]), (unsigned long long)c_fx,
                                     __ATOMIC_RELAXED, __HIP_MEMORY_SCOPE_WORKGROUP);
              __hip_atomic_fetch_add(reinterpret_cast<unsigned long long*>(&lds.tab.sum[t][1][cl]), (unsigned long long)c2_fx,
                                     __ATOMIC_RELAXED, __HIP_MEMORY_SCOPE_WORKGROUP);
              if (inside) atomic_add_slot_i64(c_img + (size_t)t * c_nimg + c_pix, c_fx);
              else
                __hip_atomic_fetch_add(reinterpret_cast<unsigned long long*>(&lds.tab.sum[t][2][cl]), (unsigned long long)c_fx,
                                       __ATOMIC_RELAXED, __HIP_MEMORY_SCOPE_WORKGROUP);
              if (Al.spectra) atomic_add_slot_i64(c_en + (size_t)t * c_ne1 + (size_t)out.e_idx, c_fx);
            } else {
              __hip_atomic_fetch_add(&lds.tab.sum[t][0][cl], c, __ATOMIC_RELAXED, __HIP_MEMORY_SCOPE_WORKGROUP);
              __hip_atomic_fetch_add(&lds.tab.sum[t][1][cl], c * c, __ATOMIC_RELAXED, __HIP_MEMORY_SCOPE_WORKGROUP);
              if (inside) unsafeAtomicAdd(c_img + (size_t)t * c_nimg + c_pix, c);
              else __hip_atomic_fetch_add(&lds.tab.sum[t][2][cl], c, __ATOMIC_RELAXED, __HIP_MEMORY_SCOPE_WORKGROUP);
              if (Al.spectra) unsafeAtomicAdd(c_en + (size_t)t * c_ne1 + (size_t)out.e_idx, c);
            }
          }
        }
      }
    }
    __builtin_amdgcn_s_setprio(0);
  };

  uint32_t chunk = (uint32_t)wave_global;
  const uint32_t lane4 = 4u * (uint32_t)lane;
  uint32_t pass = 0;
  U4 stream = U4{0u, 0u, 0u, 0u};
  for (;;) {
    const bool have_new = chunk < n_chunks;
    SART_STAGE_MARK("LOOP");
    if (have_new) {
      SART_STAGE_MARK("A0");
      if (pass == 0u) stream = stream_block(((first_chunk + (uint64_t)chunk) << 6) + (uint64_t)lane, A.seed_lo, A.seed_hi);
      const uint32_t w = word_of(stream, pass);
      const uint32_t rel = ((chunk << 8) + pass) + lane4;
      if (early_reject) {
        ZoneTable Z;
        reload_zones(Z);
        uint64_t dead_m = 0, reached_m = 0;
#pragma unroll
        for (int z = 0; z < kMaxZones; ++z) {
          const uint64_t in = ballot64(w >= Z.lo[z]) & ballot64(w <= Z.hi[z]);
          dead_m |= in;
          reached_m |= ((Z.zone_reached >> z) & 1u) ? in : 0ull;
        }
        const uint32_t chunk_lo = chunk << 8;
        uint64_t valid_m = ~0ull;
        if ((chunk_lo < rel_begin) | (chunk_lo + 256u > rel_end)) valid_m = ballot64(rel >= rel_begin) & ballot64(rel < rel_end);
        n_reached += (uint32_t)__popcll(valid_m & reached_m);
        const uint64_t mask = valid_m & ~dead_m;
        if (__builtin_amdgcn_inverse_ballot_w64(mask)) {
          const uint32_t slot = (t0 + prefix_of(mask)) % kQueue;
          Q.w[wave].ray[slot] = rel;
          Q.w[wave].u3hi[slot] = w;
        }
        t0 += (uint32_t)__popcll(mask);
      } else {
        run_phase_a(rel, (rel >= rel_begin) & (rel < rel_end), w);
      }
      pass = (pass + 1u) & 3u;
      if (pass == 0u) chunk += (uint32_t)waves_total;
      ring_sync();
    }
    if (early_reject) {
      const uint32_t n0 = t0 - h0;
      if ((n0 >= 64u) | (!have_new & (n0 > 0u))) {
        const uint32_t m = min(n0, 64u);
        const bool v = (uint32_t)lane < m;
        const uint32_t slot = (h0 + (uint32_t)lane) % kQueue;
        const uint32_t rel = Q.w[wave].ray[slot];
        const uint32_t w = Q.w[wave].u3hi[slot];
        h0 += m;
        run_phase_a(rel, v, w);
        ring_sync();
      }
    }
    const uint32_t n1 = t1 - h1;
    const bool draining = !have_new & (t0 == h0);
    if ((n1 >= 64u) | (draining & (n1 > 0u))) {
      run_phase_b(min(n1, 64u));
      ring_sync();
    }
    if (draining & (t1 == h1)) break;
  }

  SART_STAGE_MARK("EPILOGUE");
  if (A.tile_n > 0) {
    __syncthreads();
    const uint32_t tn = (uint32_t)A.tile_n, n_tile = tn * tn;
    double* const img = A.replicas + (size_t)((uint32_t)wave_global & A.replica_mask) * (size_t)A.replica_stride;
    for (uint32_t t = threadIdx.x; t < n_tile; t += BLOCK) {
      const double v = *tile_cell(t + (uint32_t)A.tile_base);
      if (__double_as_longlong(v) != 0ll) {
        const uint32_t ty = t / tn, tx = t - ty * tn;
        double* const px = &img[(size_t)((uint32_t)A.tile_y0 + ty) * (size_t)A.image_nx + ((uint32_t)A.tile_x0 + tx)];
        if constexpr (FIXED) atomic_add_slot_i64(px, __double_as_longlong(v));
        else unsafeAtomicAdd(px, v);
      }
    }
  }
  __syncthreads();
  Sum (*const red)[SART_ACC_COUNT] = reinterpret_cast<Sum (*)[SART_ACC_COUNT]>(&Q.w[0].X0[0]);
  Sum sw, sw2, sxx, syy, srr;
  if constexpr (FIXED) {
    sw = wave_sum_i64(sum_w); sw2 = wave_sum_i64(sum_w2); sxx = wave_sum_i64(sum_x); syy = wave_sum_i64(sum_y); srr = wave_sum_i64(sum_r);
  } else {
    sw = wave_sum(sum_w); sw2 = wave_sum(sum_w2); sxx = wave_sum(sum_x); syy = wave_sum(sum_y); srr = wave_sum(sum_r);
  }
  const long long swo = FIXED ? wave_sum_i64(sum_wo) : 0ll;
  const long long n_out = wave_sum_i64((long long)n_outside);
  if (lane == 0) {
    Sum* r = red[wave];
    for (int k = 0; k < SART_ACC_COUNT; ++k) r[k] = 0;
    r[SART_ACC_SUM_WEIGHTS] = sw;
    r[SART_ACC_SUM_WEIGHTS_SQ] = sw2;
    r[SART_ACC_SUM_X] = sxx;
    r[SART_ACC_SUM_Y] = syy;
    r[SART_ACC_SUM_R] = srr;
    r[SART_ACC_N_PASSED] = (Sum)n_passed;
    r[SART_ACC_N_PASSED_TILL_WINDOW] = (Sum)n_till;
    r[SART_ACC_N_HIT_NICKEL] = (Sum)n_nickel;
    r[SART_ACC_N_REACHED_TELESCOPE] = (Sum)n_reached;
    r[SART_ACC_N_SHELL_SELECTED] = (Sum)n_shell;
    r[SART_ACC_N_OUTSIDE_IMAGE] = (Sum)n_out;
    if constexpr (FIXED) r[SART_ACC_SUM_WEIGHTS_OUTSIDE] = swo;
    if constexpr (kHead) {
      lds.tab.head[wave][0] = (Sum)n_passed;
      lds.tab.head[wave][1] = sw;
// ... 1024 lines not shown
  double radial;
  LaneMasks masks;
  const uint64_t ray_id = A.ray_id_offset + i;
  bool alive;
  if (uniforms) {
    const double* u = uniforms + 6 * i;
    const Uniforms U{u[0], u[1], u[2], u[3], u[4], u[5], upper32_of_uniform(u[2])};
    alive = phase_a_core<false, -1, false>(H, P, L, U, st, sampled, reached, radial, masks);
  } else {
    const uint32_t u3_hi = word_of(stream_block(ray_id >> 2, A.seed_lo, A.seed_hi), (uint32_t)ray_id & 3u);
    alive = phase_a<false, -1, false, false, false>(H, P, L, A.seed_lo, A.seed_hi, ray_id, u3_hi, st, sampled, reached, radial, masks);
  }
  int e_idx = -1;
  if (sampled) {
    e_idx = H.test_active ? P.n_energies : sample_energy_index(HB, st.r_idx, st.u5);
    rec.emratesPre = 1.0;
    rec.energiesPre = load_energy_row(HB, e_idx).energy;
  }
  if (ballot64(alive)) {
    RayOut ro;
    if (!sampled) { st.u5 = 0.0; st.r_idx = 0; }
    phase_b<true, false, -1, false>(P, L, HB, A, st, e_idx >= 0 ? e_idx : 0, alive, ro, &rec);
  }
}

__device__ __forceinline__ void blob_to_lds(DevBlob& B, const DevBlob* __restrict__ blob) {
  const uint64_t* src = reinterpret_cast<const uint64_t*>(blob);
  uint64_t* dst = reinterpret_cast<uint64_t*>(&B);
  for (int i = threadIdx.x; i < (int)(sizeof(DevBlob) / 8); i += kRecBlock) dst[i] = src[i];
  __syncthreads();
}

__global__ __launch_bounds__(kRecBlock) void trace_records_kernel(HotA H, const DevBlob* __restrict__ blob, TraceArgs A,
                                                                   sart_axion_t* __restrict__ out, HotB HB,
                                                                   const double* __restrict__ uniforms) {
  __shared__ TablesLds S;
  __shared__ DevBlob B;
  blob_to_lds(B, blob);
  const DevParams& P = B.P;
  stage_tables<kRecBlock>(S, P, B.T);
  const LdsTables L{S.sincos, S.rcdf_hi, B.T.flux_radius_cdf, S.rguide, S.shells, S.lut};

  const uint64_t stride = (uint64_t)gridDim.x * kRecBlock;
  for (uint64_t i = (uint64_t)blockIdx.x * kRecBlock + threadIdx.x; i < A.n_rays; i += stride) {
    sart_axion_t rec = {};
    record_of_ray(H, P, L, HB, A, i, uniforms, rec);
    store_record(&out[i], rec);
  }
}

__global__ __launch_bounds__(256) void radial_verdict_kernel(HotA H, const DevBlob* __restrict__ blob, const double* __restrict__ radii, int n,
                                                             uint32_t* __restrict__ out_table, uint32_t* __restrict__ out_compares) {
  struct Lds {
    TablesLds S;
    RadialLds R;
    double behind[kRadialMarked + 1 - kRadialMax];
    DevBlob B;
  };
  __shared__ Lds lds;
  {
    const uint64_t* src = reinterpret_cast<const uint64_t*>(blob);
    uint64_t* dst = reinterpret_cast<uint64_t*>(&lds.B);
    for (int i = threadIdx.x; i < (int)(sizeof(DevBlob) / 8); i += 256) dst[i] = src[i];
    for (int i = threadIdx.x; i < kRadialMarked + 1 - kRadialMax; i += 256) lds.behind[i] = 0.0;
    __syncthreads();
  }
  const DevParams& P = lds.B.P;
  {
    const auto src = as_global(reinterpret_cast<const uint64_t*>(lds.B.T.shell_lut + kRadialTableOffset));
    uint64_t* dst = reinterpret_cast<uint64_t*>(&lds.R);
    for (int i = threadIdx.x; i < kRadialTableCells; i += 256) dst[i] = src[i];
  }
  stage_tables<256>(lds.S, P, lds.B.T, true);
  const LdsTables L{lds.S.sincos, lds.S.rcdf_hi, lds.B.T.flux_radius_cdf, lds.S.rguide, lds.S.shells, lds.S.lut, &lds.R, &lds.B.T};
  const bool cand_on = H.telescope_kind != SART_TK_LLNL;
  const int i = blockIdx.x * 256 + threadIdx.x;
  if (i < n) {
    const double radial = radii[i];
    out_table[i] = radial_verdict_table(H, P, L, cand_on, radial);
    out_compares[i] = radial_verdict_compares(H, P, L.shells, lds.B.T.shell_lut, cand_on, radial);
  }
}

__global__ __launch_bounds__(kRecBlock) void mirror_miss_count_kernel(HotA H, const DevBlob* __restrict__ blob, TraceArgs A,
                                                                       unsigned long long* __restrict__ counts) {
  __shared__ TablesLds S;
  __shared__ DevBlob B;
  blob_to_lds(B, blob);
  const DevParams& P = B.P;
  stage_tables<kRecBlock>(S, P, B.T);
  const LdsTables L{S.sincos, S.rcdf_hi, B.T.flux_radius_cdf, S.rguide, S.shells, S.lut};
  uint32_t n[5] = {0, 0, 0, 0, 0};
  const uint64_t stride = (uint64_t)gridDim.x * kRecBlock;
  const uint64_t n_round = (A.n_rays + stride - 1) / stride * stride;
  for (uint64_t i = (uint64_t)blockIdx.x * kRecBlock + threadIdx.x; i < n_round; i += stride) {
    RayState st;
    bool sampled, reached;
    double radial;
    LaneMasks masks;
    double r3sq;
    const uint64_t ray_id = A.ray_id_offset + i;
    const uint32_t u3_hi = word_of(stream_block(ray_id >> 2, A.seed_lo, A.seed_hi), (uint32_t)ray_id & 3u);
    const bool alive = phase_a<false, -1, false, false, false>(H, P, L, A.seed_lo, A.seed_hi, ray_id, u3_hi, st, sampled, reached, radial, masks, nullptr, &r3sq) &&
                       i < A.n_rays;
    const ShellDev& sh = L.shells[st.shell];
    const double X0 = st.X0, Y0 = st.Y0, tsx = st.tsx, tsy = st.tsy;
    const double Q0 = fma(X0, X0, Y0 * Y0), D0 = fma(X0, tsx, Y0 * tsy), A0 = fma(tsx, tsx, tsy * tsy);
    double z1;
    uint64_t hit1_m;
    const bool hit1 = pick_root(A0 - sh.m1_k, D0 + sh.m1_hb, Q0 - sh.m1_cc, 0.0, sh.m1_zhi, z1, hit1_m);
    const double zcb = st.zcb;
    const double m1x = fma(zcb, tsx, X0), m1y = fma(zcb, tsy, Y0);
    const double n1z = normal_z_general(P, sh, 1, m1x, m1y, zcb);
    double wx = tsx, wy = tsy, wz = 1.0, sin_a1;
    const double sin2_a1 = reflect(wx, wy, wz, 1.0 + A0, m1x, m1y, n1z, fma(m1x, m1x, fma(m1y, m1y, n1z * n1z)), sin_a1);
    const double lz = P.l_mirror - zcb, num = sh.nickel_num;
    const bool nick = sin2_a1 * fma(lz, lz, num * num) > num * num;
    const double zl = P.l_mirror, xe = fma(zl, tsx, X0), ye = fma(zl, tsy, Y0);
    const bool sure = alive & (radial > (double)P.mirror_miss_radius) & (fma(xe, xe, fma(ye, ye, kMirrorMissEps)) < r3sq) &
                      (A0 < (double)P.mirror_miss_slope_sq);
    n[0] += (uint32_t)(alive & !hit1);
    n[1] += (uint32_t)(alive & !hit1 & (st.shell > 0));
    n[2] += (uint32_t)sure;
    n[3] += (uint32_t)(sure & hit1);
    n[4] += (uint32_t)(sure & !nick);
  }
  for (int k = 0; k < 5; ++k)
    if (n[k]) atomicAdd(&counts[k], (unsigned long long)n[k]);
}

constexpr int kCompactBlock = 1024;
constexpr int kCompactMaxBlocks = 1024;
__device__ __forceinline__ uint32_t record_flags(const sart_axion_t* rec, uint32_t i, uint32_t n) {
  return i < n ? *reinterpret_cast<const uint32_t*>(rec + i) : 0u;
}
__device__ __forceinline__ void count_flag_words(uint32_t f, uint32_t* __restrict__ block_counts,
                                                 unsigned long long* __restrict__ counts) {
  __shared__ uint32_t part[kCompactBlock / 64][3];
  const int wave = threadIdx.x >> 6, lane = threadIdx.x & 63;
  const uint32_t np = (uint32_t)__popcll(ballot64((f & 0xFFu) != 0u)), nw = (uint32_t)__popcll(ballot64((f & 0xFF00u) != 0u)),
                 nn = (uint32_t)__popcll(ballot64((f & 0xFF0000u) != 0u));
  if (lane == 0) { part[wave][0] = np; part[wave][1] = nw; part[wave][2] = nn; }
  __syncthreads();
  if (threadIdx.x == 0) {
    uint32_t a = 0, b = 0, c = 0;
    for (int w = 0; w < kCompactBlock / 64; ++w) { a += part[w][0]; b += part[w][1]; c += part[w][2]; }
    block_counts[blockIdx.x] = a;
    if (b) atomicAdd(&counts[2], (unsigned long long)b);
    if (c) atomicAdd(&counts[3], (unsigned long long)c);
  }
}
__global__ __launch_bounds__(kCompactBlock) void records_count_kernel(const sart_axion_t* __restrict__ rec, uint32_t n,
                                                                       uint32_t* __restrict__ block_counts,
                                                                       unsigned long long* __restrict__ counts) {
  count_flag_words(record_flags(rec, blockIdx.x * kCompactBlock + threadIdx.x, n), block_counts, counts);
}
__global__ __launch_bounds__(kCompactMaxBlocks) void records_scan_kernel(uint32_t* __restrict__ block_counts, uint32_t n_blocks,
                                                                          unsigned long long* __restrict__ block_first,
                                                                          unsigned long long* __restrict__ counts, uint32_t n) {
  __shared__ uint32_t wave_sum[kCompactMaxBlocks / 64];
  const int wave = threadIdx.x >> 6, lane = threadIdx.x & 63;
  const uint32_t v = threadIdx.x < n_blocks ? block_counts[threadIdx.x] : 0u;
  uint32_t incl = v;
#pragma unroll
  for (int d = 1; d < 64; d <<= 1) {
    const uint32_t o = (uint32_t)__shfl_up((int)incl, d, 64);
// ... 444 lines not shown
                     static_cast<FixedCheck*>(check_dev));
}

void launch_finalize_channels(const void* in, double* out, int n_channels, int n_energies1, int spectra, size_t n_img, double q_w,
                              double q_w2, void* check_dev, hipStream_t stream) {
  FinalizeChannelsArgs F{n_channels, n_energies1, spectra, 0, (long long)n_img, q_w, q_w2};
  hipLaunchKernelGGL(finalize_channels_kernel, dim3(n_channels), dim3(256), 0, stream, reinterpret_cast<const long long*>(in), out, F,
                     static_cast<FixedCheck*>(check_dev));
}
void launch_channel_fractions(const double* rates_dev, const double* total_dev, double* frac_dev, int n_channels, int stride,
                              size_t n_cells, unsigned long long* first_bad_dev, hipStream_t stream) {
  (void)hipMemsetAsync(first_bad_dev, 0xFF, sizeof(unsigned long long), stream);
  hipLaunchKernelGGL(channel_fractions_kernel, dim3((unsigned)((n_cells + 255) / 256)), dim3(256), 0, stream, rates_dev, total_dev,
                     frac_dev, n_channels, stride, (long long)n_cells, first_bad_dev);
}

size_t fixed_check_bytes() { return sizeof(FixedCheck); }
std::string fixed_check_describe(const void* host_copy) {
  const FixedCheck& C = *static_cast<const FixedCheck*>(host_copy);
  const char* names[5] = {"pixels", "SUM_WEIGHTS - outside", "radial bins", "energy bins", "SUM_WEIGHTS"};
  std::string s = " [quanta as lo + hi x 2^40:";
  for (int i = 0; i < 5; ++i) {
    if ((i == 2 || i == 3) && !C.spectra) continue;
    long long lo = C.fail[2 * i], hi = C.fail[2 * i + 1];
    limbs_normalise(lo, hi);
    s += std::string(i ? "," : "") + " " + names[i] + " " + std::to_string(lo) + " + " + std::to_string(hi);
  }
  return s + "]";
}
void launch_rollover_fixed(void* acc, void* hi, size_t n, void* check_dev, hipStream_t stream) {
  hipLaunchKernelGGL(rollover_fixed_kernel, dim3((unsigned)((n + 255) / 256)), dim3(256), 0, stream, static_cast<long long*>(acc),
                     static_cast<long long*>(hi), (long long)n, static_cast<FixedCheck*>(check_dev));
}
void launch_finalize_fixed(const void* in, const void* hi, double* out, size_t n_img, int spectra, int n_radial_bins, int n_energies1, double q_w,
                           double q_w2, double q_pos, double q_refl, void* check_dev, hipStream_t stream) {
  FinalizeArgs F{(long long)n_img, spectra, n_radial_bins, n_energies1, 0, q_w, q_w2, q_pos, q_refl};
  const size_t total = n_img + SART_ACC_COUNT + (spectra ? 2 * (size_t)n_radial_bins + 3 * (size_t)n_energies1 : 0);
  FixedCheck* const C = static_cast<FixedCheck*>(check_dev);
  (void)hipMemsetAsync(reinterpret_cast<char*>(C) + 8, 0, offsetof(FixedCheck, fail) - 8, stream);
  hipLaunchKernelGGL(finalize_fixed_kernel, dim3((unsigned)((total + 255) / 256)), dim3(256), 0, stream,
                     reinterpret_cast<const long long*>(in), reinterpret_cast<const long long*>(hi), out, F, C);
  hipLaunchKernelGGL(fixed_check_kernel, dim3(1), dim3(1), 0, stream, C);
}
void launch_finalize_scan(const void* in, double* out, int n_masses, const double* q_w, const double* q_w2, int shared_row,
                          void* check_dev, hipStream_t stream, uint32_t counter_slots) {
  FinalizeScanArgs F;
  memset(&F, 0, sizeof F);
  F.n_masses = n_masses;
  F.shared_row = shared_row;
  F.counter_slots = counter_slots;
  for (int k = 0; k < n_masses; ++k) { F.q_w[k] = q_w[k]; F.q_w2[k] = q_w2[k]; }
  hipLaunchKernelGGL(finalize_scan_kernel, dim3(1), dim3(64), 0, stream, reinterpret_cast<const long long*>(in), out, F, static_cast<FixedCheck*>(check_dev));
}
void launch_finalize_scan_bands(const void* rows, const void* shared_row, const void* in, double* out, const void* counts_in, double* counts_out,
                                int n_masses, int n_cells, const double* q_w, const double* q_w2, void* check_dev, hipStream_t stream) {
  FinalizeBandsArgs F;
  memset(&F, 0, sizeof F);
  F.n_masses = n_masses;
  F.n_cells = n_cells;
  for (int k = 0; k < n_masses; ++k) { F.q_w[k] = q_w[k]; F.q_w2[k] = q_w2[k]; }
  hipLaunchKernelGGL(finalize_scan_bands_kernel, dim3(n_masses + (counts_in ? 1 : 0)), dim3(64), 0, stream, static_cast<const long long*>(rows),
                     static_cast<const long long*>(shared_row), static_cast<const long long*>(in), out, static_cast<const long long*>(counts_in),
                     counts_out, F, static_cast<FixedCheck*>(check_dev));
}
int compact_chunk_max() { return kCompactBlock * kCompactMaxBlocks; }
void launch_compact_records(const sart_axion_t* rec, uint32_t n, sart_axion_t* out, unsigned long long capacity, uint32_t* block_counts,
                            unsigned long long* block_first, unsigned long long* counts, hipStream_t stream) {
  const uint32_t n_blocks = (n + kCompactBlock - 1) / kCompactBlock;
  hipLaunchKernelGGL(records_count_kernel, dim3(n_blocks), dim3(kCompactBlock), 0, stream, rec, n, block_counts, counts);
  hipLaunchKernelGGL(records_scan_kernel, dim3(1), dim3(kCompactMaxBlocks), 0, stream, block_counts, n_blocks, block_first, counts, n);
  hipLaunchKernelGGL(records_scatter_kernel, dim3(n_blocks), dim3(kCompactBlock), 0, stream, rec, n, block_first, out, capacity);
}
void launch_trace_records(const HotA& H, const HotB& HB, const DevBlob* blob, const TraceArgs& A, sart_axion_t* out, int n_blocks,
                          hipStream_t stream, const double* uniforms_dev) {
  hipLaunchKernelGGL(trace_records_kernel, dim3(n_blocks), dim3(kRecBlock), 0, stream, H, blob, A, out, HB, uniforms_dev);
}
void launch_mirror_miss_count(const HotA& H, const DevBlob* blob, const TraceArgs& A, unsigned long long* counts, int n_blocks, hipStream_t stream) {
  hipLaunchKernelGGL(mirror_miss_count_kernel, dim3(n_blocks), dim3(kRecBlock), 0, stream, H, blob, A, counts);
}
void launch_radial_verdicts(const HotA& H, const DevBlob* blob, const double* radii, int n, uint32_t* out_table, uint32_t* out_compares,
                            hipStream_t stream) {
  hipLaunchKernelGGL(radial_verdict_kernel, dim3((n + 255) / 256), dim3(256), 0, stream, H, blob, radii, n, out_table, out_compares);
}
void launch_stage_columns(const HotA& H, const HotB& HB, const DevBlob* blob, const TraceArgs& A, uint64_t* stage, uint32_t* flags,
                          uint32_t mask, int n_blocks, hipStream_t stream) {
  hipLaunchKernelGGL(columns_stage_kernel, dim3(n_blocks), dim3(kRecBlock), 0, stream, H, blob, A, stage, flags, HB, mask);
}
void launch_compact_columns(const uint64_t* stage, const uint32_t* flags, uint32_t n, uint32_t mask, unsigned long long ray_id0, uint64_t* out,
                            unsigned long long capacity, uint32_t* block_counts, unsigned long long* block_first,
                            unsigned long long* counts, hipStream_t stream) {
  const uint32_t n_blocks = (n + kCompactBlock - 1) / kCompactBlock;
  hipLaunchKernelGGL(columns_count_kernel, dim3(n_blocks), dim3(kCompactBlock), 0, stream, flags, n, block_counts, counts);
  hipLaunchKernelGGL(records_scan_kernel, dim3(1), dim3(kCompactMaxBlocks), 0, stream, block_counts, n_blocks, block_first, counts, n);
  hipLaunchKernelGGL(columns_scatter_kernel, dim3(n_blocks), dim3(kCompactBlock), 0, stream, stage, flags, n, block_first, out, capacity, mask,
                     ray_id0);
}

}
```

### solaraxionraytracing_amd/csrc/sart_trace_histogram.inc

```
  struct LdsLayout {
    TablesLds S;
    RadialLds R;
    double tile_extra[kTileExtraCells];
    DevBlob B;
    TraceArgs Ab;
    QueueLds<BLOCK / 64, HistRings> Q;
  };
  static_assert(sizeof(RadialLds) % 8 == 0 && (kRadialMarked + 1) * sizeof(double) <= sizeof(RadialLds) + kTileExtraCells * sizeof(double),
                "entry kRadialMarked of either column lies in the table or in the tile's cells");
  __shared__ LdsLayout lds;
  TablesLds& S = lds.S;
  QueueLds<BLOCK / 64, HistRings>& Q = lds.Q;
  static_assert(!PATHC || (FAST && !ROT && GAS >= 0), "the constant-path form belongs to the unrotated specialisations");
  static_assert(!SCAN || GAS != 0, "a mass scan needs the gas stage");
  static_assert(!SCAN || kScanMaxMasses * 2 * kScanLanes <= (BLOCK / 64) * kQueue, "the scan accumulators live in the image tile's 128 doubles per wave");
  __shared__ uint32_t scan_zero[kScanMaxMasses];
  static_assert(!BANDS || SCAN, "the bands belong to the mass scan");
  __shared__ uint32_t scan_band_n[BANDS ? kScanLanes : 1];
  static_assert((BLOCK / 64) * kQueue == kTileRingCells && kImageTileMax * kImageTileMax <= kTileRingCells + kTileExtraCells &&
                    kImageTileExtraMax * kImageTileExtraMax <= kTileExtraCells && BLOCK / 64 == kTileRingCells / kQueue,
                "the LDS image tile (host: kImageTileMax): 128 doubles per wave of this workgroup's rings + the cells behind the tables");
  static_assert((offsetof(LdsLayout, Q) % 512) == 0, "the rings are addressed with ds_*2st64 offsets (units of 512 bytes for 64-bit columns)");
  auto tile_cell_lo = [&](uint32_t t) -> double* {
    return PATHC ? &Q.w[t >> 7].path[t & 127u] : reinterpret_cast<double*>(&Q.w[t >> 7].ray[0]) + (t & 127u);
  };
  auto tile_cell = [&](uint32_t t) -> double* {
    return t < (uint32_t)kTileRingCells ? tile_cell_lo(t) : &lds.tile_extra[t - (uint32_t)kTileRingCells];
  };
  DevBlob& B = lds.B;
  TraceArgs& Ab = lds.Ab;
  {
    const uint64_t* src = reinterpret_cast<const uint64_t*>(blob);
    uint64_t* dst = reinterpret_cast<uint64_t*>(&B);
    for (int i = threadIdx.x; i < (int)(sizeof(DevBlob) / 8); i += BLOCK) dst[i] = src[i];
    if (threadIdx.x == 0) Ab = A;
    __syncthreads();
  }
  const DevParams& Pb = B.P;
  const DevTables& Tb = B.T;
  {
    uint64_t* q = reinterpret_cast<uint64_t*>(&Q);
    for (int i = threadIdx.x; i < (int)(sizeof(Q) / 8); i += BLOCK) q[i] = 0ull;
    for (int i = threadIdx.x; i < kTileExtraCells; i += BLOCK) lds.tile_extra[i] = 0.0;
    if (SCAN && threadIdx.x < kScanMaxMasses) scan_zero[threadIdx.x] = 0u;
    if (BANDS && threadIdx.x < kScanLanes) scan_band_n[threadIdx.x] = 0u;
  }
  constexpr bool RTAB = FAST;
  if (RTAB && H.radial_table) {
    const auto src = as_global(reinterpret_cast<const uint64_t*>(Tb.shell_lut + kRadialTableOffset));
    uint64_t* dst = reinterpret_cast<uint64_t*>(&lds.R);
    for (int i = threadIdx.x; i < kRadialTableCells; i += BLOCK) dst[i] = src[i];
  }
  stage_tables<BLOCK>(S, Pb, Tb, RTAB && H.radial_table);
  const LdsTables L{S.sincos, S.rcdf_hi, Tb.flux_radius_cdf, S.rguide, S.shells, S.lut, &lds.R, &Tb};

  const int lane = threadIdx.x & 63;
  const int wave = __builtin_amdgcn_readfirstlane((int)(threadIdx.x >> 6));
  const uint64_t waves_total = (uint64_t)gridDim.x * (BLOCK / 64);
  const uint64_t wave_global = (uint64_t)blockIdx.x * (BLOCK / 64) + wave;
  const bool early_reject = (SCAN && !PATHC) ? false : H.n_zones > 0;
  const uint64_t first_chunk = A.ray_id_offset >> 8;
  uint64_t id_base = first_chunk << 8;
  asm volatile("" : "+s"(id_base));
  const uint32_t rel_begin = (uint32_t)(A.ray_id_offset & 255u);
  const uint32_t rel_end = rel_begin + (uint32_t)A.n_rays;
  const uint32_t n_chunks = (rel_end + 255u) >> 8;

  uint32_t n_reached = 0, n_shell = 0, n_nickel = 0, n_till = 0, n_passed = 0;
  uint32_t n_outside = 0;
  using Sum = std::conditional_t<FIXED, long long, double>;
  Sum sum_w = 0, sum_w2 = 0, sum_x = 0, sum_y = 0, sum_r = 0;
  long long sum_wo = 0;
#ifdef SART_STAGE_TIMING
  uint64_t cyc_a0 = 0, cyc_a1 = 0, cyc_b = 0, cyc_bs[6] = {0, 0, 0, 0, 0, 0};
#endif
  uint32_t h0 = 0, t0 = 0;
  uint32_t h1 = 0, t1 = 0;

  auto ring_sync = [] {
    __builtin_amdgcn_fence(__ATOMIC_RELEASE, "wavefront");
    __builtin_amdgcn_wave_barrier();
    __builtin_amdgcn_fence(__ATOMIC_ACQUIRE, "wavefront");
  };
  auto prefix_from = [](uint64_t mask, uint32_t base) {
    return __builtin_amdgcn_mbcnt_hi((uint32_t)(mask >> 32), __builtin_amdgcn_mbcnt_lo((uint32_t)mask, base));
  };

  constexpr bool HOLD_SINCOS = SART_A_SINCOS_VGPR && FAST && GAS == 0 && !SCAN;
  SinCosCoef Ksc = {-0.5992645293207921, 2.5501640398773455, -5.16771278004997, 3.141592653589793, -1.3352627688545895, 4.0587121264167685,
                    -4.934802200544679};
  if constexpr (HOLD_SINCOS) asm volatile("" : "+v"(Ksc.s3), "+v"(Ksc.s2), "+v"(Ksc.s1), "+v"(Ksc.s0), "+v"(Ksc.d3), "+v"(Ksc.d2), "+v"(Ksc.d1));
  auto run_phase_a = [&](uint32_t rel, bool valid, uint32_t u3_hi) {
    SART_STAGE_MARK("A1");
    __builtin_amdgcn_s_setprio(SART_PRIO_A1);
    RayState st;
    bool sampled = false, reached = false;
    double radial;
    HotA Hl;
    reload_hot(Hl);
    constexpr bool ZEXT = FAST && !ROT && GAS >= 0;
    LaneMasks M;
    double r3sq = 0.0;
    (void)phase_a<FAST, ROT ? 1 : 0, ZEXT, PATHC, true, RTAB>(Hl, Pb, L, A.seed_lo, A.seed_hi, id_base + (uint64_t)rel, u3_hi, st, sampled, reached, radial,
                                                              M, HOLD_SINCOS ? &Ksc : nullptr, ROT ? nullptr : &r3sq);
    const uint64_t valid_m = ballot64(valid);
    n_reached += (uint32_t)__popcll(valid_m & M.reached);
    const uint64_t selected = valid_m & M.ok;
    n_shell += (uint32_t)__popcll(selected);
    uint64_t sure = 0ull;
    const uint64_t cand = (ROT || Hl.telescope_kind == SART_TK_LLNL) ? 0ull
                                                                     : (selected & (RTAB ? M.cand : ballot64(radial > (double)Pb.mirror_miss_radius)));
    if (cand) {
      if (RTAB && Hl.radial_table) r3sq = L.shells[st.shell].n1_r3sq;
      const double zl = Pb.l_mirror, xe = fma(zl, st.tsx, st.X0), ye = fma(zl, st.tsy, st.Y0);
      sure = cand & ballot64(fma(xe, xe, fma(ye, ye, kMirrorMissEps)) < r3sq) &
             ballot64(fma(st.tsx, st.tsx, st.tsy * st.tsy) < (double)Pb.mirror_miss_slope_sq);
      n_nickel += (uint32_t)__popcll(sure);
    }
#ifdef SART_DEBUG_KNOBS
    const uint64_t mask = (A.flags & 0x10000000u) ? 0ull : (selected & (RTAB ? M.keep : ~ballot64(radial < Pb.shell0_miss_radius)) & ~sure);
#else
    const uint64_t mask = selected & (RTAB ? M.keep : ~ballot64(radial < Pb.shell0_miss_radius)) & ~sure;
#endif
    const bool alive = __builtin_amdgcn_inverse_ballot_w64(mask);
    const uint32_t cnt = (uint32_t)__popcll(mask);
    if (alive) {
      asm volatile("; hot: ring 1 write");
      const uint32_t slot = prefix_from(mask, t1) % kQueue;
      Q.w[wave].X0[slot] = st.X0; Q.w[wave].Y0[slot] = st.Y0;
      Q.w[wave].tsx[slot] = st.tsx; Q.w[wave].tsy[slot] = st.tsy;
      if (!PATHC) Q.w[wave].path[slot] = st.path_cb;
      Q.w[wave].cell[slot] = make_uint2((uint32_t)(st.r_idx | (st.shell << 16)), st.u5_hi);
    }
    t1 += cnt;
    __builtin_amdgcn_s_setprio(0);
  };

  auto run_phase_b = [&](uint32_t n_valid) {
    SART_STAGE_MARK("B");
    __builtin_amdgcn_s_setprio(SART_PRIO_B);
    RayState st;
    const bool valid = (uint32_t)lane < n_valid;
    const uint32_t slot = (h1 + (uint32_t)lane) % kQueue;
    RayOut out;
    {
      st.X0 = Q.w[wave].X0[slot]; st.Y0 = Q.w[wave].Y0[slot];
      st.tsx = Q.w[wave].tsx[slot]; st.tsy = Q.w[wave].tsy[slot];
      st.path_cb = PATHC ? H.length_b : Q.w[wave].path[slot];
      const uint2 cell = Q.w[wave].cell[slot];
      st.u5 = u52(cell.y, 0u);
      st.u5_hi = cell.y;
      if (!ROT) {
        st.zcb = -(H.dz3 - H.dz1);
      } else {
        st.zcb = zcb_rotated(Pb.rx_s, -Pb.rx_c * Pb.ry_s, Pb.rx_c * Pb.ry_c, Pb.half_length_telescope, st.X0 + Pb.entrance_x,
                             st.Y0 + Pb.entrance_y, st.tsx, st.tsy, H.dz3 - H.dz1);
      }
      const int packed = (int)cell.x;
      st.r_idx = packed & 0xFFFF;
      st.shell = packed >> 16;
      const DevBlob& Bo = lds_opaque(B);
      HotB HB;
      reload_kernarg(HB, offsetof(HistKernArgs, HB));
      asm volatile("" :: "s"(HB.cdf_hi32), "s"(HB.energy_guide), "s"(HB.energy_tab), "s"(HB.refl), "s"(HB.refl_n_angles), "s"(HB.cdf_stride));
      phase_b<false, FAST, GAS, FAST && !ROT && GAS >= 0, SCAN>(Bo.P, L, HB, lds_opaque(Ab), st, (!FAST && H.test_active) ? Pb.n_energies : -1, valid, out, nullptr);
      if constexpr (SCAN) {
        SART_STAGE_MARK("SCAN");
        n_passed += (uint32_t)__popcll(out.m_passed);
        struct { int32_t n_masses, pad; } hdr;
        reload_kernarg(hdr, offsetof(HistKernArgs, SC));
        const uint32_t fl = (uint32_t)__builtin_amdgcn_readfirstlane((int)Ab.flags);
        const bool use_prob = !(fl & SART_CF_IGNORE_CONV_PROB) & ((GAS >= 0) ? (GAS == 1) : (__builtin_amdgcn_readfirstlane(Bo.P.stage_gas) != 0));
        const double term1 = Bo.P.gas_term1;
        const GasCos cos_lead = GasCos::make();
        uint32_t cell = 0u;
        if constexpr (BANDS) {
          struct { int32_t e0; uint32_t mul; } b0;
          struct { uint32_t window, unused; } b1;
          reload_kernarg(b0, offsetof(HistKernArgs, SC) + offsetof(ScanArgs, m) + offsetof(ScanMass, aux));
          reload_kernarg(b1, offsetof(HistKernArgs, SC) + offsetof(ScanArgs, m) + sizeof(ScanMass) + offsetof(ScanMass, aux));
          const uint32_t d = (uint32_t)(out.e_idx - b0.e0);
          cell = (d < b1.window ? __umulhi(2u * d + 1u, b0.mul) : (uint32_t)hdr.pad) & (kScanLanes - 1u);
          if (__builtin_amdgcn_inverse_ballot_w64(out.m_passed))
            __hip_atomic_fetch_add(&scan_band_n[cell], 1u, __ATOMIC_RELAXED, __HIP_MEMORY_SCOPE_WORKGROUP);
        }
        for (int k = 0; k < hdr.n_masses; ++k) {
          asm volatile("; hot: per-mass loop of the fused scan");
          ScanMass M;
          reload_kernarg(M, offsetof(HistKernArgs, SC) + offsetof(ScanArgs, m) + (size_t)k * sizeof(ScanMass));
          double w = out.weight;
          if (use_prob) w *= gas_conversion_prob(M.dm2_abs, out.gas, term1, L.sincos, cos_lead);
          const uint64_t nz = out.m_passed & ballot64(w != 0.0);
          if (nz != out.m_passed) {
            asm volatile("; rare: a conversion probability of exactly zero");
            if (lane == 0) atomicAdd(&scan_zero[k], (uint32_t)__popcll(out.m_passed & ~nz));
          }
          if (__builtin_amdgcn_inverse_ballot_w64(nz)) {
            const uint32_t t = (uint32_t)k * (2u * kScanLanes) + (BANDS ? cell : ((uint32_t)lane & (kScanLanes - 1u)));
            if constexpr (FIXED) {
              __hip_atomic_fetch_add(reinterpret_cast<unsigned long long*>(tile_cell_lo(t)), (unsigned long long)to_fixed(w, M.fx_scale_w),
                                     __ATOMIC_RELAXED, __HIP_MEMORY_SCOPE_WORKGROUP);
              __hip_atomic_fetch_add(reinterpret_cast<unsigned long long*>(tile_cell_lo(t + kScanLanes)), (unsigned long long)to_fixed(w * w, M.fx_scale_w2),
                                     __ATOMIC_RELAXED, __HIP_MEMORY_SCOPE_WORKGROUP);
            } else {
              __hip_atomic_fetch_add(tile_cell_lo(t), w, __ATOMIC_RELAXED, __HIP_MEMORY_SCOPE_WORKGROUP);
              __hip_atomic_fetch_add(tile_cell_lo(t + kScanLanes), w * w, __ATOMIC_RELAXED, __HIP_MEMORY_SCOPE_WORKGROUP);
            }
          }
        }
      }
    }
    h1 += n_valid;
    if constexpr (SCAN) {
      n_nickel += (uint32_t)__popcll(out.m_nickel);
      __builtin_amdgcn_s_setprio(0);
      return;
    }
    __builtin_amdgcn_s_setprio(SART_PRIO_ACC);
#ifdef SART_STAGE_TIMING
    for (int k = 0; k < 5; ++k) cyc_bs[k] += out.tb[k + 1] - out.tb[k];
    cyc_bs[5] += out.tb[0];
#endif
    n_nickel += (uint32_t)__popcll(out.m_nickel);
    n_till += (uint32_t)__popcll(out.m_till);
    n_passed += (uint32_t)__popcll(out.m_passed);
    if (out.passed) {
      SART_STAGE_MARK("ACC");
      TraceArgs Al;
      reload_kernarg(Al, offsetof(HistKernArgs, A));
      asm volatile("" :: "s"(Al.replicas), "s"(Al.replica_mask), "s"(Al.replica_stride), "s"(Al.image_nx), "s"(Al.image_ny),
                   "s"(Al.image_x_min), "s"(Al.image_y_min), "s"(Al.image_inv_step_x), "s"(Al.image_inv_step_y), "s"(Al.spectra),
                   "s"(Al.tile_x0), "s"(Al.tile_y0), "s"(Al.tile_n), "s"(Al.tile_base));
      long long w_fx = 0;
      if constexpr (FIXED) {
        w_fx = to_fixed(out.weight, Al.fx_scale_w);
        sum_w += w_fx;
        sum_w2 += to_fixed(out.weight * out.weight, Al.fx_scale_w2);
        sum_x += to_fixed(out.px, kFixedPositionScale);
        sum_y += to_fixed(out.py, kFixedPositionScale);
        sum_r += to_fixed(out.rdet, kFixedPositionScale);
      } else {
        sum_w += out.weight;
        sum_w2 = fma(out.weight, out.weight, sum_w2);
        sum_x += out.px;
        sum_y += out.py;
        sum_r += out.rdet;
      }
      const double fx = (out.px - Al.image_x_min) * Al.image_inv_step_x;
      const double fy = (out.py - Al.image_y_min) * Al.image_inv_step_y;
      const int nx = Al.image_nx, ny = Al.image_ny;
      const uint64_t inside_m = ballot64(fx >= 0.0) & ballot64(fx < (double)nx) & ballot64(fy >= 0.0) & ballot64(fy < (double)ny);
      const bool inside = __builtin_amdgcn_inverse_ballot_w64(inside_m);
      n_outside += inside ? 0u : 1u;
      if constexpr (FIXED) {
        if (out.m_passed & ~inside_m) {
          asm volatile("; rare: passed rays outside the image");
          sum_wo += inside ? 0ll : w_fx;
        }
      }
#ifdef SART_DEBUG_KNOBS
      const uint32_t rep_key = (Al.flags & 0x08000000u) ? blockIdx.x : (uint32_t)wave_global;
      double* const img = Al.replicas + (size_t)(rep_key & Al.replica_mask) * (size_t)Al.replica_stride;
#else
      double* const img = Al.replicas + (size_t)((uint32_t)wave_global & Al.replica_mask) * (size_t)Al.replica_stride;
#endif
#ifdef SART_DEBUG_KNOBS
      if (inside && !(Al.flags & 0x40000000u))
#else
      if (inside)
#endif
      {
        const uint32_t ix = (uint32_t)(int)fx, iy = (uint32_t)(int)fy;
        const uint32_t tn = (uint32_t)Al.tile_n;
        const uint32_t tx = ix - (uint32_t)Al.tile_x0, ty = iy - (uint32_t)Al.tile_y0;
        if ((tx < tn) & (ty < tn)) {
          const uint32_t t = ty * tn + tx + (uint32_t)Al.tile_base;
          if constexpr (FIXED)
            __hip_atomic_fetch_add(reinterpret_cast<unsigned long long*>(tile_cell(t)), (unsigned long long)w_fx, __ATOMIC_RELAXED,
                                   __HIP_MEMORY_SCOPE_WORKGROUP);
          else
            __hip_atomic_fetch_add(tile_cell(t), out.weight, __ATOMIC_RELAXED, __HIP_MEMORY_SCOPE_WORKGROUP);
        } else {
          const uint32_t pix = iy * (uint32_t)nx + ix;
          typedef __attribute__((address_space(1))) char* gbytes;
          if constexpr (FIXED) atomic_add_slot_i64((double*)((gbytes)img + pix * 8u), w_fx);
          else unsafeAtomicAdd((double*)((gbytes)img + pix * 8u), out.weight);
        }
      }
      if (Al.spectra) {
        double* rad = acc + (size_t)nx * (size_t)ny + SART_ACC_COUNT;
        double* en = rad + 2 * (size_t)Al.n_radial_bins;
        const size_t ne1 = (size_t)Pb.n_energies + 1;
        const int rb = min((int)(out.rdet * Al.radial_inv_bin), Al.n_radial_bins - 1);
        if constexpr (FIXED) {
          atomic_add_slot_i64(&rad[rb], 1);
          atomic_add_slot_i64(&rad[(size_t)Al.n_radial_bins + rb], w_fx);
          atomic_add_slot_i64(&en[out.e_idx], 1);
          atomic_add_slot_i64(&en[ne1 + out.e_idx], w_fx);
          atomic_add_slot_i64(&en[2 * ne1 + out.e_idx], to_fixed(out.reflect, kFixedReflectScale));
        } else {
          unsafeAtomicAdd(&rad[rb], 1.0);
          unsafeAtomicAdd(&rad[(size_t)Al.n_radial_bins + rb], out.weight);
          unsafeAtomicAdd(&en[out.e_idx], 1.0);
          unsafeAtomicAdd(&en[ne1 + out.e_idx], out.weight);
          unsafeAtomicAdd(&en[2 * ne1 + out.e_idx], out.reflect);
        }
      }
    }
    __builtin_amdgcn_s_setprio(0);
  };

  constexpr bool kZonesInVgprs = FAST;
  uint32_t zone_lo_v[kMaxZones], zone_hi_v[kMaxZones];
#pragma unroll
  for (int z = 0; z < kMaxZones; ++z) {
    zone_lo_v[z] = H.zone_lo[z];
    zone_hi_v[z] = H.zone_hi[z];
    if (kZonesInVgprs) asm volatile("" : "+v"(zone_lo_v[z]), "+v"(zone_hi_v[z]));
  }
  uint32_t zone_reached_v = H.zone_reached;
  if (kZonesInVgprs) asm volatile("" : "+v"(zone_reached_v));
  uint32_t chunk = (uint32_t)wave_global;
  const uint32_t lane4 = 4u * (uint32_t)lane;
  uint32_t pass = 0;
  U4 stream = U4{0u, 0u, 0u, 0u};
#ifdef SART_STAGE_TIMING
  const uint64_t cyc_start = __builtin_readcyclecounter();
  const uint64_t real_start = __builtin_amdgcn_s_memrealtime();
#define SART_STAMP(var) const uint64_t var = __builtin_readcyclecounter()
#define SART_SPAN(acc, t_begin) acc += __builtin_readcyclecounter() - (t_begin)
#else
#define SART_STAMP(var)
#define SART_SPAN(acc, t_begin)
#endif
  for (;;) {
    const bool have_new = chunk < n_chunks;
    SART_STAGE_MARK("LOOP");
    if (have_new) {
      SART_STAGE_MARK("A0");
      SART_STAMP(ts_a0);
      if (pass == 0u) {
        asm volatile("; hot x0.25: one block of the shared word stream per four passes");
        stream = stream_block(((first_chunk + (uint64_t)chunk) << 6) + (uint64_t)lane, A.seed_lo, A.seed_hi);
      }
      const uint32_t w = stream.x;
      stream.x = stream.y; stream.y = stream.z; stream.z = stream.w;
      const uint32_t rel = ((chunk << 8) + pass) + lane4;
      if (early_reject) {
        ZoneTable Z;
        if constexpr (!kZonesInVgprs) reload_zones(Z);
        const uint32_t zone_reached = kZonesInVgprs ? (uint32_t)__builtin_amdgcn_readfirstlane((int)zone_reached_v) : Z.zone_reached;
        struct WordMasks { uint64_t mask, reached; };
        auto a0_masks = [&](uint32_t ww, uint32_t rr, uint32_t zr, uint32_t ck) -> WordMasks {
          uint64_t dead_m = 0, in_first = 0;
#pragma unroll
          for (int z = 0; z < kMaxZones; ++z) {
            const uint64_t in = kZonesInVgprs ? (ballot64(ww >= zone_lo_v[z]) & ballot64(ww <= zone_hi_v[z]))
                                              : (ballot64(ww >= Z.lo[z]) & ballot64(ww <= Z.hi[z]));
            dead_m |= in;
            if (z == 0) in_first = in;
          }
          const uint64_t reached_m = dead_m & ~((zr & 1u) ? 0ull : in_first);
          uint64_t valid_m = ~0ull;
          if (ck - 1u >= n_chunks - 2u) valid_m = ballot64(rr >= rel_begin) & ballot64(rr < rel_end);
#ifdef SART_DEBUG_KNOBS
          const uint64_t mask = (A.flags & 0x20000000u) ? 0ull : (valid_m & ~dead_m);
#else
          const uint64_t mask = valid_m & ~dead_m;
#endif
          return WordMasks{mask, valid_m & reached_m};
        };
        auto ring0_push = [&](uint64_t mask, uint32_t ww, uint32_t rr) {
          if (__builtin_amdgcn_inverse_ballot_w64(mask)) {
            asm volatile("; hot: ring 0 write");
            const uint32_t slot = prefix_from(mask, t0) % kQueue;
            Q.w[wave].ray[slot] = rr;
            Q.w[wave].u3hi[slot] = ww;
          }
          t0 += (uint32_t)__popcll(mask);
        };
        const WordMasks wa = a0_masks(w, rel, zone_reached, chunk);
        n_reached += (uint32_t)__popcll(wa.reached);
        ring0_push(wa.mask, w, rel);
        if ((zone_reached >> (pass + (uint32_t)kA0WideBit)) & 1u) {
          uint32_t zr = zone_reached, ck = chunk;
          asm volatile("" : "+s"(zr), "+s"(ck));
          const uint32_t wb = stream.x;
          const WordMasks mb = a0_masks(wb, rel + 1u, zr, ck);
          if ((t0 - h0) + (uint32_t)__popcll(mb.mask) <= (uint32_t)kQueue) {
            n_reached += (uint32_t)__popcll(mb.reached);
            ring0_push(mb.mask, wb, rel + 1u);
            stream.x = stream.y; stream.y = stream.z; stream.z = stream.w;
            pass += 1u;
          }
        }
      } else {
        run_phase_a(rel, (rel >= rel_begin) & (rel < rel_end), w);
      }
      pass = (pass + 1u) & 3u;
      if (pass == 0u) chunk += (uint32_t)waves_total;
      ring_sync();
      SART_SPAN(cyc_a0, ts_a0);
    }
    SART_STAGE_MARK("LOOP");
    if (early_reject) {
      const uint32_t n0 = t0 - h0;
      bool a1_due = n0 >= 64u;
      if (chunk >= n_chunks) {
        asm volatile("; the drain");
        a1_due = n0 > 0u;
      }
      if (a1_due) {
        const uint32_t m = min(n0, 64u);
        const bool v = (uint32_t)lane < m;
        const uint32_t slot = (h0 + (uint32_t)lane) % kQueue;
        const uint32_t rel = Q.w[wave].ray[slot];
        const uint32_t w = Q.w[wave].u3hi[slot];
        h0 += m;
        SART_STAMP(ts_a1);
        run_phase_a(rel, v, w);
        ring_sync();
        SART_SPAN(cyc_a1, ts_a1);
      }
    }
    SART_STAGE_MARK("LOOP");
    const uint32_t n1 = t1 - h1;
    bool b_due = n1 >= 64u, draining = false;
    if (chunk >= n_chunks) {
      asm volatile("; the drain");
      draining = t0 == h0;
      b_due |= draining & (n1 > 0u);
    }
    if (b_due) {
      SART_STAMP(ts_b);
      run_phase_b(min(n1, 64u));
      ring_sync();
      SART_SPAN(cyc_b, ts_b);
    }
    if (draining) {
      asm volatile("; the drain");
      if (t1 == h1) break;
    }
  }

// ... 81 lines not shown
```

Baseline: 111.0 billion.

## Use single-compare zone ranges and trim integer ops in trace histogram kernels

```diff
diff --git a/solaraxionraytracing_amd/csrc/sart_angular_scan.inc b/solaraxionraytracing_amd/csrc/sart_angular_scan.inc
--- a/solaraxionraytracing_amd/csrc/sart_angular_scan.inc
+++ b/solaraxionraytracing_amd/csrc/sart_angular_scan.inc
@@ -234,12 +234,12 @@
   };
 
   constexpr bool kZonesInVgprs = FAST;
-  uint32_t zone_lo_v[kMaxZones], zone_hi_v[kMaxZones];
+  uint32_t zone_lo_v[kMaxZones], zone_aux_v[kMaxZones];
 #pragma unroll
   for (int z = 0; z < kMaxZones; ++z) {
     zone_lo_v[z] = H.zone_lo[z];
-    zone_hi_v[z] = H.zone_hi[z];
-    if (kZonesInVgprs) asm volatile("" : "+v"(zone_lo_v[z]), "+v"(zone_hi_v[z]));
+    zone_aux_v[z] = zone_aux_of(H.zone_lo[z], H.zone_n[z]);
+    if (kZonesInVgprs) asm volatile("" : "+v"(zone_lo_v[z]), "+v"(zone_aux_v[z]));
   }
   uint32_t zone_reached_v = H.zone_reached;
   if (kZonesInVgprs) asm volatile("" : "+v"(zone_reached_v));
@@ -262,14 +262,14 @@
           ZoneTable Z;
           if constexpr (!kZonesInVgprs) reload_zones(Z);
           const uint32_t zone_reached = kZonesInVgprs ? (uint32_t)__builtin_amdgcn_readfirstlane((int)zone_reached_v) : Z.zone_reached;
-          uint64_t dead_m = 0, reached_m = 0;
-#pragma unroll
-          for (int z = 0; z < kMaxZones; ++z) {
-            const uint64_t in = kZonesInVgprs ? (ballot64(w >= zone_lo_v[z]) & ballot64(w <= zone_hi_v[z]))
-                                              : (ballot64(w >= Z.lo[z]) & ballot64(w <= Z.hi[z]));
-            dead_m |= in;
-            reached_m |= ((zone_reached >> z) & 1u) ? in : 0ull;
+          if constexpr (!kZonesInVgprs) {
+#pragma unroll
+            for (int z = 0; z < kMaxZones; ++z) Z.n[z] = zone_aux_of(Z.lo[z], Z.n[z]);
           }
+          uint64_t in[kMaxZones], reached_m = 0;
+          const uint64_t dead_m = kZonesInVgprs ? zone_masks(w, zone_lo_v, zone_aux_v, in) : zone_masks(w, Z.lo, Z.n, in);
+#pragma unroll
+          for (int z = 0; z < kMaxZones; ++z) reached_m |= ((zone_reached >> z) & 1u) ? in[z] : 0ull;
           const uint64_t valid_m = ballot64(rel >= rel_begin) & ballot64(rel < rel_end);
           n_reached += (uint32_t)__popcll(valid_m & reached_m);
           const uint64_t mask = valid_m & ~dead_m;
diff --git a/solaraxionraytracing_amd/csrc/sart_api.hip b/solaraxionraytracing_amd/csrc/sart_api.hip
--- a/solaraxionraytracing_amd/csrc/sart_api.hip
+++ b/solaraxionraytracing_amd/csrc/sart_api.hip
@@ -69,6 +69,7 @@
 void launch_mirror_miss_count(const HotA& H, const DevBlob* blob, const TraceArgs& A, unsigned long long* counts, int n_blocks, hipStream_t stream);
 void launch_radial_verdicts(const HotA& H, const DevBlob* blob, const double* radii, int n, uint32_t* out_table, uint32_t* out_compares,
                             hipStream_t stream);
+void launch_zone_ranges(const HotA& H, const uint32_t* words, uint32_t* out, hipStream_t stream);
 int records_block();
 int compact_chunk_max();
 void launch_compact_records(const sart_axion_t* rec, uint32_t n, sart_axion_t* out, unsigned long long capacity, uint32_t* block_counts,
@@ -714,7 +715,7 @@
 void build_zones(const sart_setup_t& s, const DevParams& P, int n_radii, HotA& h, double tilt_max) {
   h.n_zones = 0;
   h.zone_reached = 0;
-  for (int z = 0; z < kMaxZones; ++z) { h.zone_lo[z] = 1u; h.zone_hi[z] = 0u; }
+  for (int z = 0; z < kMaxZones; ++z) { h.zone_lo[z] = 1u; h.zone_n[z] = 0u; }
   if (P.test_active || n_radii < 1) return;
   const double R = P.radius_cb;
   const double r_sun_max = (0.0015 + (n_radii - 1) * 0.0005) * P.sun_radius;
@@ -753,8 +754,10 @@
     const double ulo = std::min(1.0, (z.lo / R) * (z.lo / R)), uhi = std::min(1.0, (z.hi / R) * (z.hi / R));
     const double wlo = std::ceil(ulo * 4294967296.0) + 1.0, whi = std::floor(uhi * 4294967296.0) - 2.0;
     if (!(whi >= wlo)) continue;
-    h.zone_lo[h.n_zones] = static_cast<uint32_t>(std::min(wlo, 4294967295.0));
-    h.zone_hi[h.n_zones] = static_cast<uint32_t>(std::min(whi, 4294967295.0));
+    const uint32_t lo = static_cast<uint32_t>(std::min(wlo, 4294967295.0)), hi = static_cast<uint32_t>(std::min(whi, 4294967295.0));
+    if (hi < lo) continue;
+    h.zone_lo[h.n_zones] = lo;
+    h.zone_n[h.n_zones] = hi - lo + 1u;
     if (z.reached) h.zone_reached |= (1u << h.n_zones);
     h.n_zones++;
   }
@@ -762,7 +765,7 @@
 
 double a0_survival_of(const HotA& h) {
   double covered = 0.0;
-  for (int z = 0; z < h.n_zones; ++z) covered += static_cast<double>(h.zone_hi[z]) - static_cast<double>(h.zone_lo[z]) + 1.0;
+  for (int z = 0; z < h.n_zones; ++z) covered += static_cast<double>(h.zone_n[z]);
   return std::min(1.0, std::max(0.0, 1.0 - covered / 4294967296.0));
 }
 
@@ -1537,9 +1540,44 @@
 __attribute__((visibility("default"))) int sart_internal_zones(sart_context* c, uint32_t* lo, uint32_t* hi, uint32_t* reached_bits) {
   if (!c || !lo || !hi || !reached_bits) return -1;
   if (hipSetDevice(c->device) != hipSuccess || refresh_derived(c) != 0 || sync_blob(c) != 0) return -1;
-  for (int z = 0; z < c->hot.n_zones; ++z) { lo[z] = c->hot.zone_lo[z]; hi[z] = c->hot.zone_hi[z]; }
+  for (int z = 0; z < c->hot.n_zones; ++z) { lo[z] = c->hot.zone_lo[z]; hi[z] = c->hot.zone_lo[z] + (c->hot.zone_n[z] - 1u); }
   *reached_bits = c->hot.zone_reached & ((1u << kMaxZones) - 1u);
   return c->hot.n_zones;
+}
+
+__attribute__((visibility("default"))) int sart_internal_zone_counts(sart_context* c, uint32_t* lo, uint32_t* n) {
+  if (!c || !lo || !n) return -1;
+  if (hipSetDevice(c->device) != hipSuccess || refresh_derived(c) != 0 || sync_blob(c) != 0) return -1;
+  for (int z = 0; z < kMaxZones; ++z) { lo[z] = c->hot.zone_lo[z]; n[z] = c->hot.zone_n[z]; }
+  return c->hot.n_zones;
+}
+__attribute__((visibility("default"))) int sart_internal_zone_verdicts(sart_context* c, const uint32_t* words, int32_t n, uint32_t* out,
+                                                                       const uint32_t* table_lo, const uint32_t* table_n, uint32_t table_reached) {
+  if (!c || !words || !out || n < 1 || n > 256 || (table_lo && !table_n)) return fail(SART_ERR_INVALID_ARGUMENT, "invalid argument");
+  SART_HIP(hipSetDevice(c->device));
+  if (int rc = refresh_derived(c)) return rc;
+  if (int rc = sync_blob(c)) return rc;
+  HotA h = c->hot;
+  if (table_lo) {
+    for (int z = 0; z < kMaxZones; ++z) {
+      if (static_cast<uint64_t>(table_lo[z]) + table_n[z] > 4294967296ull) return fail(SART_ERR_INVALID_ARGUMENT, "a zone wraps");
+      h.zone_lo[z] = table_lo[z];
+      h.zone_n[z] = table_n[z];
+    }
+    h.zone_reached = table_reached & ((1u << kMaxZones) - 1u);
+  }
+  uint32_t padded[256] = {};
+  std::copy(words, words + n, padded);
+  DevBuf<uint32_t> d_w, d_out;
+  if (int rc = d_w.upload(padded, 256)) return rc;
+  if (int rc = d_out.resize(256)) return rc;
+  launch_zone_ranges(h, d_w.p, d_out.p, c->stream);
+  SART_HIP(hipGetLastError());
+  uint32_t got[256];
+  SART_HIP(hipMemcpyAsync(got, d_out.p, sizeof(got), hipMemcpyDeviceToHost, c->stream));
+  SART_HIP(hipStreamSynchronize(c->stream));
+  std::copy(got, got + n, out);
+  return 0;
 }
 
 __attribute__((visibility("default"))) double sart_internal_a0_wide_share(double survival) { return a0_wide_fallback_share(survival); }
@@ -1984,6 +2022,7 @@
     if (c->tile.in_pilot) R = 64;
     if (p->image_nx == 0) R = 1;
     while (R & (R - 1)) R &= R - 1;
+    while (R > 1 && static_cast<uint64_t>(R) * (static_cast<uint64_t>(p->image_nx) * static_cast<uint64_t>(p->image_ny) + 32u) * 8u > 0xFFFFFFFFull) R >>= 1;
     if (R > 1) {
       const size_t n_img = static_cast<size_t>(p->image_nx) * static_cast<size_t>(p->image_ny);
       const size_t pad = 32;
diff --git a/solaraxionraytracing_amd/csrc/sart_device.h b/solaraxionraytracing_amd/csrc/sart_device.h
--- a/solaraxionraytracing_amd/csrc/sart_device.h
+++ b/solaraxionraytracing_amd/csrc/sart_device.h
@@ -108,7 +108,7 @@
   int32_t n_shells, lut_n, radial_table, inner_blocks;
   int32_t n_zones;
   uint32_t zone_reached;
-  uint32_t zone_lo[4], zone_hi[4];
+  uint32_t zone_lo[4], zone_n[4];
 };
 constexpr int kMaxZones = 4;
 constexpr int kA0WideBit = 8;
diff --git a/solaraxionraytracing_amd/csrc/sart_kernels.hip b/solaraxionraytracing_amd/csrc/sart_kernels.hip
--- a/solaraxionraytracing_amd/csrc/sart_kernels.hip
+++ b/solaraxionraytracing_amd/csrc/sart_kernels.hip
@@ -7,6 +7,31 @@
 #include "../../include/sart.h"
 #include "sart_device.h"
 #include "sart_math.h"
+
+#ifndef SART_A0_ZONE_RANGE
+#define SART_A0_ZONE_RANGE 1
+#endif
+#ifndef SART_A0_FIRST_ROUND
+#define SART_A0_FIRST_ROUND 1
+#endif
+#ifndef SART_A_WORD_SHIFTS
+#define SART_A_WORD_SHIFTS 1
+#endif
+#ifndef SART_A_SHELL_MUL24
+#define SART_A_SHELL_MUL24 1
+#endif
+#ifndef SART_ACC_BOUNDS_UINT
+#define SART_ACC_BOUNDS_UINT 1
+#endif
+#ifndef SART_ACC_REPLICA_VGPR
+#define SART_ACC_REPLICA_VGPR 1
+#endif
+#ifndef SART_ACC_MUL24
+#define SART_ACC_MUL24 1
+#endif
+#ifndef SART_ACC_CELL_SELECT
+#define SART_ACC_CELL_SELECT 1
+#endif
 
 namespace sart {
 
@@ -31,7 +56,11 @@
 }
 
 __device__ __forceinline__ U4 stream_block(uint64_t group, uint32_t k0, uint32_t k1) {
-  return philox4x32((uint32_t)group, (uint32_t)(group >> 32), 3u, 0u, k0, k1);
+  uint32_t c1 = (uint32_t)(group >> 32);
+#if SART_A0_FIRST_ROUND
+  asm("" : "+v"(c1));
+#endif
+  return philox4x32((uint32_t)group, c1, 3u, 0u, k0, k1);
 }
 __device__ __forceinline__ uint32_t word_of(const U4& b, uint32_t k) {
   return k == 0u ? b.x : (k == 1u ? b.y : (k == 2u ? b.z : b.w));
@@ -40,6 +69,12 @@
 #define SART_STAGE_MARK(name) asm volatile("; SART_STAGE " name)
 
 __device__ __forceinline__ uint64_t ballot64(bool pred) { return __builtin_amdgcn_ballot_w64(pred); }
+
+__device__ __forceinline__ uint32_t cvt_i32_sat(double f) {
+  uint32_t i;
+  asm("v_cvt_i32_f64 %0, %1" : "=v"(i) : "v"(f));
+  return i;
+}
 
 template <uint64_t BITS>
 __device__ __forceinline__ double scalar_const() {
@@ -813,7 +848,10 @@
 
 __device__ __forceinline__ Uniforms uniforms_of(uint32_t seed_lo, uint32_t seed_hi, uint64_t ray_id, uint32_t u3_hi) {
   const uint32_t id_lo = (uint32_t)ray_id, id_hi = (uint32_t)(ray_id >> 32);
-  const U4 b0 = philox4x32(id_lo, id_hi, 0u, 0u, seed_lo, seed_hi);
+  U4 b0 = philox4x32(id_lo, id_hi, 0u, 0u, seed_lo, seed_hi);
+#if SART_A_WORD_SHIFTS
+  asm("" : "+v"(b0.y), "+v"(b0.w));
+#endif
   Uniforms U;
   U.u2 = u52(b0.x, 0u);
   U.u2_hi = b0.x;
@@ -1229,8 +1267,23 @@
 struct ZoneTable {
   int32_t n_zones;
   uint32_t zone_reached;
-  uint32_t lo[kMaxZones], hi[kMaxZones];
+  uint32_t lo[kMaxZones], n[kMaxZones];
 };
+__device__ __forceinline__ uint32_t zone_aux_of(uint32_t lo, uint32_t n) { return SART_A0_ZONE_RANGE ? n : lo + n - 1u; }
+__device__ __forceinline__ uint64_t zone_masks(uint32_t w, const uint32_t (&lo)[kMaxZones], const uint32_t (&aux)[kMaxZones],
+                                               uint64_t (&in)[kMaxZones]) {
+  uint64_t dead_m = 0;
+#pragma unroll
+  for (int z = 0; z < kMaxZones; ++z) {
+#if SART_A0_ZONE_RANGE
+    in[z] = ballot64(w - lo[z] < aux[z]);
+#else
+    in[z] = ballot64(w >= lo[z]) & ballot64(w <= aux[z]);
+#endif
+    dead_m |= in[z];
+  }
+  return dead_m;
+}
 static_assert(sizeof(ZoneTable) == sizeof(HotA) - offsetof(HotA, n_zones), "ZoneTable mirrors the tail of HotA");
 static_assert(offsetof(WaveRings, u3hi) == offsetof(WaveRings, ray) + kQueue * sizeof(uint32_t) && offsetof(WaveRings, ray) % 8 == 0 &&
                   offsetof(HistRings, u3hi) == offsetof(HistRings, ray) + kQueue * sizeof(uint32_t) && offsetof(HistRings, ray) % 8 == 0,
@@ -1754,13 +1807,13 @@
       if (early_reject) {
         ZoneTable Z;
         reload_zones(Z);
-        uint64_t dead_m = 0, reached_m = 0;
+        uint32_t aux[kMaxZones];
+        uint64_t in[kMaxZones], reached_m = 0;
 #pragma unroll
-        for (int z = 0; z < kMaxZones; ++z) {
-          const uint64_t in = ballot64(w >= Z.lo[z]) & ballot64(w <= Z.hi[z]);
-          dead_m |= in;
-          reached_m |= ((Z.zone_reached >> z) & 1u) ? in : 0ull;
-        }
+        for (int z = 0; z < kMaxZones; ++z) aux[z] = zone_aux_of(Z.lo[z], Z.n[z]);
+        const uint64_t dead_m = zone_masks(w, Z.lo, aux, in);
+#pragma unroll
+        for (int z = 0; z < kMaxZones; ++z) reached_m |= ((Z.zone_reached >> z) & 1u) ? in[z] : 0ull;
         const uint32_t chunk_lo = chunk << 8;
         uint64_t valid_m = ~0ull;
         if ((chunk_lo < rel_begin) | (chunk_lo + 256u > rel_end)) valid_m = ballot64(rel >= rel_begin) & ballot64(rel < rel_end);
@@ -2951,6 +3004,22 @@
   }
 }
 
+__global__ __launch_bounds__(256) void zone_ranges_kernel(HotA H, const uint32_t* __restrict__ words, uint32_t* __restrict__ out) {
+  uint32_t lo[kMaxZones], aux[kMaxZones];
+#pragma unroll
+  for (int z = 0; z < kMaxZones; ++z) {
+    lo[z] = H.zone_lo[z];
+    aux[z] = zone_aux_of(H.zone_lo[z], H.zone_n[z]);
+    asm volatile("" : "+v"(lo[z]), "+v"(aux[z]));
+  }
+  uint64_t in[kMaxZones], reached_m = 0;
+  const uint64_t dead_m = zone_masks(words[threadIdx.x], lo, aux, in);
+#pragma unroll
+  for (int z = 0; z < kMaxZones; ++z) reached_m |= ((H.zone_reached >> z) & 1u) ? in[z] : 0ull;
+  const uint32_t lane = threadIdx.x & 63u;
+  out[threadIdx.x] = (uint32_t)((dead_m >> lane) & 1ull) | ((uint32_t)((reached_m >> lane) & 1ull) << 1);
+}
+
 __global__ __launch_bounds__(kRecBlock) void mirror_miss_count_kernel(HotA H, const DevBlob* __restrict__ blob, TraceArgs A,
                                                                        unsigned long long* __restrict__ counts) {
   __shared__ TablesLds S;
@@ -3561,6 +3630,9 @@
                             hipStream_t stream) {
   hipLaunchKernelGGL(radial_verdict_kernel, dim3((n + 255) / 256), dim3(256), 0, stream, H, blob, radii, n, out_table, out_compares);
 }
+void launch_zone_ranges(const HotA& H, const uint32_t* words, uint32_t* out, hipStream_t stream) {
+  hipLaunchKernelGGL(zone_ranges_kernel, dim3(1), dim3(256), 0, stream, H, words, out);
+}
 void launch_stage_columns(const HotA& H, const HotB& HB, const DevBlob* blob, const TraceArgs& A, uint64_t* stage, uint32_t* flags,
                           uint32_t mask, int n_blocks, hipStream_t stream) {
   hipLaunchKernelGGL(columns_stage_kernel, dim3(n_blocks), dim3(kRecBlock), 0, stream, H, blob, A, stage, flags, HB, mask);
diff --git a/solaraxionraytracing_amd/csrc/sart_trace_histogram.inc b/solaraxionraytracing_amd/csrc/sart_trace_histogram.inc
--- a/solaraxionraytracing_amd/csrc/sart_trace_histogram.inc
+++ b/solaraxionraytracing_amd/csrc/sart_trace_histogram.inc
@@ -27,6 +27,18 @@
   auto tile_cell = [&](uint32_t t) -> double* {
     return t < (uint32_t)kTileRingCells ? tile_cell_lo(t) : &lds.tile_extra[t - (uint32_t)kTileRingCells];
   };
+  auto tile_cell_acc = [&](uint32_t t) -> double* {
+    if constexpr (!SART_ACC_CELL_SELECT && !SART_ACC_MUL24) {
+      return tile_cell(t);
+    } else {
+      const uint32_t wave_off = SART_ACC_MUL24 ? __umul24(t >> 7, (uint32_t)sizeof(HistRings)) : (t >> 7) * (uint32_t)sizeof(HistRings);
+      const uint32_t ring = (uint32_t)(offsetof(LdsLayout, Q) + (PATHC ? offsetof(HistRings, path) : offsetof(HistRings, ray))) + wave_off + (t & 127u) * 8u;
+      const uint32_t extra = (uint32_t)offsetof(LdsLayout, tile_extra) + (t - (uint32_t)kTileRingCells) * 8u;
+      char* const base = reinterpret_cast<char*>(&lds);
+      if constexpr (SART_ACC_CELL_SELECT) return reinterpret_cast<double*>(base + (t < (uint32_t)kTileRingCells ? ring : extra));
+      else return t < (uint32_t)kTileRingCells ? reinterpret_cast<double*>(base + ring) : reinterpret_cast<double*>(base + extra);
+    }
+  };
   DevBlob& B = lds.B;
   TraceArgs& Ab = lds.Ab;
   {
@@ -90,6 +102,16 @@
   SinCosCoef Ksc = {-0.5992645293207921, 2.5501640398773455, -5.16771278004997, 3.141592653589793, -1.3352627688545895, 4.0587121264167685,
                     -4.934802200544679};
   if constexpr (HOLD_SINCOS) asm volatile("" : "+v"(Ksc.s3), "+v"(Ksc.s2), "+v"(Ksc.s1), "+v"(Ksc.s0), "+v"(Ksc.d3), "+v"(Ksc.d2), "+v"(Ksc.d1));
+#ifdef SART_DEBUG_KNOBS
+  constexpr bool HOLD_REPLICA = false;
+#else
+  constexpr bool HOLD_REPLICA = SART_ACC_REPLICA_VGPR && FAST && GAS == 0 && !SCAN && !FIXED;
+#endif
+  uint32_t replica_off_v = 0u;
+  if constexpr (HOLD_REPLICA) {
+    replica_off_v = ((uint32_t)wave_global & A.replica_mask) * A.replica_stride * 8u;
+    asm volatile("" : "+v"(replica_off_v));
+  }
   auto run_phase_a = [&](uint32_t rel, bool valid, uint32_t u3_hi) {
     SART_STAGE_MARK("A1");
     __builtin_amdgcn_s_setprio(SART_PRIO_A1);
@@ -111,7 +133,12 @@
     const uint64_t cand = (ROT || Hl.telescope_kind == SART_TK_LLNL) ? 0ull
                                                                      : (selected & (RTAB ? M.cand : ballot64(radial > (double)Pb.mirror_miss_radius)));
     if (cand) {
-      if (RTAB && Hl.radial_table) r3sq = L.shells[st.shell].n1_r3sq;
+      if (RTAB && Hl.radial_table) {
+        if constexpr (SART_A_SHELL_MUL24)
+          r3sq = *reinterpret_cast<const double*>(reinterpret_cast<const char*>(L.shells) + __mul24(st.shell, (int)sizeof(ShellDev)) + offsetof(ShellDev, n1_r3sq));
+        else
+          r3sq = L.shells[st.shell].n1_r3sq;
+      }
       const double zl = Pb.l_mirror, xe = fma(zl, st.tsx, st.X0), ye = fma(zl, st.tsy, st.Y0);
       sure = cand & ballot64(fma(xe, xe, fma(ye, ye, kMirrorMissEps)) < r3sq) &
              ballot64(fma(st.tsx, st.tsx, st.tsy * st.tsy) < (double)Pb.mirror_miss_slope_sq);
@@ -249,7 +276,15 @@
       const double fx = (out.px - Al.image_x_min) * Al.image_inv_step_x;
       const double fy = (out.py - Al.image_y_min) * Al.image_inv_step_y;
       const int nx = Al.image_nx, ny = Al.image_ny;
-      const uint64_t inside_m = ballot64(fx >= 0.0) & ballot64(fx < (double)nx) & ballot64(fy >= 0.0) & ballot64(fy < (double)ny);
+      uint32_t ix = 0u, iy = 0u;
+      uint64_t inside_m;
+      if constexpr (SART_ACC_BOUNDS_UINT) {
+        ix = cvt_i32_sat(floor(fx));
+        iy = cvt_i32_sat(floor(fy));
+        inside_m = ballot64(ix < (uint32_t)nx) & ballot64(iy < (uint32_t)ny) & ballot64(!__builtin_isunordered(fx, fy));
+      } else {
+        inside_m = ballot64(fx >= 0.0) & ballot64(fx < (double)nx) & ballot64(fy >= 0.0) & ballot64(fy < (double)ny);
+      }
       const bool inside = __builtin_amdgcn_inverse_ballot_w64(inside_m);
       n_outside += inside ? 0u : 1u;
       if constexpr (FIXED) {
@@ -262,7 +297,7 @@
       const uint32_t rep_key = (Al.flags & 0x08000000u) ? blockIdx.x : (uint32_t)wave_global;
       double* const img = Al.replicas + (size_t)(rep_key & Al.replica_mask) * (size_t)Al.replica_stride;
 #else
-      double* const img = Al.replicas + (size_t)((uint32_t)wave_global & Al.replica_mask) * (size_t)Al.replica_stride;
+      double* const img = HOLD_REPLICA ? Al.replicas : Al.replicas + (size_t)((uint32_t)wave_global & Al.replica_mask) * (size_t)Al.replica_stride;
 #endif
 #ifdef SART_DEBUG_KNOBS
       if (inside && !(Al.flags & 0x40000000u))
@@ -270,21 +305,23 @@
       if (inside)
 #endif
       {
-        const uint32_t ix = (uint32_t)(int)fx, iy = (uint32_t)(int)fy;
+        if constexpr (!SART_ACC_BOUNDS_UINT) { ix = (uint32_t)(int)fx; iy = (uint32_t)(int)fy; }
         const uint32_t tn = (uint32_t)Al.tile_n;
         const uint32_t tx = ix - (uint32_t)Al.tile_x0, ty = iy - (uint32_t)Al.tile_y0;
         if ((tx < tn) & (ty < tn)) {
-          const uint32_t t = ty * tn + tx + (uint32_t)Al.tile_base;
+          const uint32_t t = (SART_ACC_MUL24 ? __umul24(ty, tn) : ty * tn) + tx + (uint32_t)Al.tile_base;
+          double* const cell = tile_cell_acc(t);
           if constexpr (FIXED)
-            __hip_atomic_fetch_add(reinterpret_cast<unsigned long long*>(tile_cell(t)), (unsigned long long)w_fx, __ATOMIC_RELAXED,
+            __hip_atomic_fetch_add(reinterpret_cast<unsigned long long*>(cell), (unsigned long long)w_fx, __ATOMIC_RELAXED,
                                    __HIP_MEMORY_SCOPE_WORKGROUP);
           else
-            __hip_atomic_fetch_add(tile_cell(t), out.weight, __ATOMIC_RELAXED, __HIP_MEMORY_SCOPE_WORKGROUP);
+            __hip_atomic_fetch_add(cell, out.weight, __ATOMIC_RELAXED, __HIP_MEMORY_SCOPE_WORKGROUP);
         } else {
           const uint32_t pix = iy * (uint32_t)nx + ix;
           typedef __attribute__((address_space(1))) char* gbytes;
-          if constexpr (FIXED) atomic_add_slot_i64((double*)((gbytes)img + pix * 8u), w_fx);
-          else unsafeAtomicAdd((double*)((gbytes)img + pix * 8u), out.weight);
+          const uint32_t byte = HOLD_REPLICA ? pix * 8u + replica_off_v : pix * 8u;
+          if constexpr (FIXED) atomic_add_slot_i64((double*)((gbytes)img + byte), w_fx);
+          else unsafeAtomicAdd((double*)((gbytes)img + byte), out.weight);
         }
       }
       if (Al.spectra) {
@@ -311,12 +348,12 @@
   };
 
   constexpr bool kZonesInVgprs = FAST;
-  uint32_t zone_lo_v[kMaxZones], zone_hi_v[kMaxZones];
+  uint32_t zone_lo_v[kMaxZones], zone_aux_v[kMaxZones];
 #pragma unroll
   for (int z = 0; z < kMaxZones; ++z) {
     zone_lo_v[z] = H.zone_lo[z];
-    zone_hi_v[z] = H.zone_hi[z];
-    if (kZonesInVgprs) asm volatile("" : "+v"(zone_lo_v[z]), "+v"(zone_hi_v[z]));
+    zone_aux_v[z] = zone_aux_of(H.zone_lo[z], H.zone_n[z]);
+    if (kZonesInVgprs) asm volatile("" : "+v"(zone_lo_v[z]), "+v"(zone_aux_v[z]));
   }
   uint32_t zone_reached_v = H.zone_reached;
   if (kZonesInVgprs) asm volatile("" : "+v"(zone_reached_v));
@@ -348,18 +385,17 @@
       const uint32_t rel = ((chunk << 8) + pass) + lane4;
       if (early_reject) {
         ZoneTable Z;
-        if constexpr (!kZonesInVgprs) reload_zones(Z);
+        if constexpr (!kZonesInVgprs) {
+          reload_zones(Z);
+#pragma unroll
+          for (int z = 0; z < kMaxZones; ++z) Z.n[z] = zone_aux_of(Z.lo[z], Z.n[z]);
+        }
         const uint32_t zone_reached = kZonesInVgprs ? (uint32_t)__builtin_amdgcn_readfirstlane((int)zone_reached_v) : Z.zone_reached;
         struct WordMasks { uint64_t mask, reached; };
         auto a0_masks = [&](uint32_t ww, uint32_t rr, uint32_t zr, uint32_t ck) -> WordMasks {
-          uint64_t dead_m = 0, in_first = 0;
-#pragma unroll
-          for (int z = 0; z < kMaxZones; ++z) {
-            const uint64_t in = kZonesInVgprs ? (ballot64(ww >= zone_lo_v[z]) & ballot64(ww <= zone_hi_v[z]))
-                                              : (ballot64(ww >= Z.lo[z]) & ballot64(ww <= Z.hi[z]));
-            dead_m |= in;
-            if (z == 0) in_first = in;
-          }
+          uint64_t in[kMaxZones];
+          const uint64_t dead_m = kZonesInVgprs ? zone_masks(ww, zone_lo_v, zone_aux_v, in) : zone_masks(ww, Z.lo, Z.n, in);
+          const uint64_t in_first = in[0];
           const uint64_t reached_m = dead_m & ~((zr & 1u) ? 0ull : in_first);
           uint64_t valid_m = ~0ull;
           if (ck - 1u >= n_chunks - 2u) valid_m = ballot64(rr >= rel_begin) & ballot64(rr < rel_end);
```

Result: no change. 111.8 billion (median of 6 runs) (+0.8%).
